# RDG0818/MAZero

Hardware: NVIDIA B200
Metric: mcts_sims_per_sec (higher is better)
Workload: dtype bf16

## Files before the change

### mazero_b200/csrc/infer_hmma.cuh

```cuda
#pragma once
#include <cuda_bf16.h>

#include "../../include/maz_infer.h"
#include "umma.cuh"

namespace maz {
namespace hmma {

using namespace umma;

constexpr int H = 128, NHEAD = 8, HD = 16, GH = 64, PH = 32, SUP = 11, NLAYER = 3;
constexpr int NCHUNK = MAZ_INFER_NCHUNK, NSLOT = 3;
constexpr int TM = 32;
#ifndef MAZ_HMMA_NQ
#define MAZ_HMMA_NQ 4
#endif
constexpr int NQ = MAZ_HMMA_NQ;
constexpr int NT = H / NQ / 8;
constexpr int GT = GH / NQ / 8;
constexpr int CW = H / NQ, FW = GH / NQ;
static_assert(NQ == 4 || NQ == 8, "NQ");
constexpr int NCONS = 64 * NQ, NTHREADS = NCONS + 32;
constexpr int PAD = 8;
constexpr int LDA = (H + PAD) * 2;
constexpr int LDQ = (3 * H + PAD) * 2;
constexpr int LDP = (PH + PAD) * 2;
constexpr int LDO = (48 + PAD) * 2;
constexpr int LDG = GH + 4;
constexpr int LDV = GH + 4;
constexpr uint32_t SLOT_BYTES = 128 * (H + PAD) * 2;
#ifndef MAZ_HMMA_PIECE
#define MAZ_HMMA_PIECE 4352
#endif
constexpr uint32_t PIECE = MAZ_HMMA_PIECE;
#ifndef MAZ_GEMM_UNROLL
#define MAZ_GEMM_UNROLL 2
#endif
constexpr int GEMM_UNROLL = MAZ_GEMM_UNROLL;

constexpr uint32_t OFF_X = 0;
constexpr uint32_t OFF_T = OFF_X + TM * LDA;
constexpr uint32_t OFF_HH = OFF_T + TM * LDA;
constexpr uint32_t OFF_ONE = OFF_HH + TM * LDA;
constexpr uint32_t OFF_PH = OFF_ONE + TM * LDO;
constexpr uint32_t OFF_Q = OFF_PH + TM * LDP;
constexpr uint32_t OFF_STAT = OFF_Q + TM * LDQ;
constexpr uint32_t STAT_SET = TM * NQ * 8;
constexpr uint32_t OFF_VP = OFF_STAT + 3 * TM * NQ * 8;
constexpr uint32_t OFF_ROW = OFF_VP + 2 * SUP * LDV * 4;
constexpr uint32_t OFF_W = ((OFF_ROW + TM * 16 + 127) / 128) * 128;
constexpr uint32_t OFF_P = OFF_W + NSLOT * SLOT_BYTES;
constexpr int G_R = 0, G_V = TM * LDG;
constexpr int Y_R = 0, Y_V = TM * GH;
constexpr int PL0 = 2 * TM * LDG;
static_assert((PL0 + TM * 48) * 4 <= TM * LDQ, "heads scratch must fit in the q|k|v region");
static_assert(2 * TM * GH * 4 <= 2 * TM * LDA, "layer-2 features must fit in the X + T tiles");

using Desc = ::maz_infer_desc;

struct RowInfo { int root, agent, valid, r0; };

__device__ __forceinline__ int tile_rpt(const Desc &d) { return d.roots_per_tile > 0 ? d.roots_per_tile : TM / d.N; }

struct SimIo {
    const int *idx_x;
    const int *actions;
    float *reward, *value, *probs, *beta;
    int root0;
    float *next_hidden;
    int *greedy;
    float *logits_out;
};
__device__ __forceinline__ SimIo io_from_desc(const Desc &d)
{
    return SimIo{d.idx_x, d.actions, d.reward, d.value, d.probs, d.beta, 0, d.next_hidden, d.greedy, d.logits_out};
}

__host__ __device__ inline size_t smem_bytes(int vec_floats) { return (size_t)OFF_P + (size_t)vec_floats * 4 + 128; }

#define HSM_DECL extern __shared__ __align__(128) uint8_t hsm[]
__device__ __forceinline__ uint32_t sbase()
{
    HSM_DECL;
    return smem_u32(hsm);
}

__device__ __forceinline__ void ldsm4(uint32_t addr, uint32_t (&r)[4])
{
    asm volatile("ldmatrix.sync.aligned.m8n8.x4.shared.b16 {%0,%1,%2,%3}, [%4];" : "=r"(r[0]), "=r"(r[1]), "=r"(r[2]), "=r"(r[3]) : "r"(addr));
}
__device__ __forceinline__ void mma16816(float (&c)[4], const uint32_t (&a)[4], uint32_t b0, uint32_t b1)
{
    asm volatile("mma.sync.aligned.m16n8k16.row.col.f32.bf16.bf16.f32 {%0,%1,%2,%3}, {%4,%5,%6,%7}, {%8,%9}, {%0,%1,%2,%3};"
                 : "+f"(c[0]), "+f"(c[1]), "+f"(c[2]), "+f"(c[3])
                 : "r"(a[0]), "r"(a[1]), "r"(a[2]), "r"(a[3]), "r"(b0), "r"(b1));
}
__device__ __forceinline__ uint32_t pack2(float a, float b)
{
    __nv_bfloat162 p = __floats2bfloat162_rn(a, b);
    return *reinterpret_cast<uint32_t *>(&p);
}
__device__ __forceinline__ void sts32(uint32_t saddr, uint32_t v) { asm volatile("st.shared.b32 [%0], %1;" ::"r"(saddr), "r"(v) : "memory"); }
__device__ __forceinline__ float2 ldp2(uint32_t saddr)
{
    float2 v;
    asm("ld.shared.v2.f32 {%0,%1}, [%2];" : "=f"(v.x), "=f"(v.y) : "r"(saddr));
    return v;
}
__device__ __forceinline__ float4 lds4v(uint32_t saddr)
{
    float4 v;
    asm volatile("ld.shared.v4.f32 {%0,%1,%2,%3}, [%4];" : "=f"(v.x), "=f"(v.y), "=f"(v.z), "=f"(v.w) : "r"(saddr) : "memory");
    return v;
}

struct Thr {
    int lane, warp, g, t, mt, nq, rA, rB;
    uint32_t a_off, w_off;
    __device__ __forceinline__ Thr()
    {
        const int tid = threadIdx.x;
        lane = tid & 31; warp = tid >> 5; g = lane >> 2; t = lane & 3; mt = warp & 1; nq = warp >> 1;
        rA = 16 * mt + g; rB = rA + 8;
        a_off = (uint32_t)(16 * mt + (lane & 7) + ((lane >> 3) & 1) * 8);
        w_off = (uint32_t)((lane & 7) + (lane >> 4) * 8);
    }
    __device__ __forceinline__ uint32_t a_addr(uint32_t tile, int lda) const { return tile + a_off * lda + (uint32_t)(lane >> 4) * 16u; }
    __device__ __forceinline__ uint32_t w_addr(uint32_t slot, int ldw, int n0) const
    {
        return slot + (uint32_t)(n0 + w_off) * ldw + (uint32_t)((lane >> 3) & 1) * 16u;
    }
};

template <int NT, int KS>
__device__ __forceinline__ void gemm_fixed(float (&acc)[NT][4], const Thr &th, uint32_t a_tile, int lda, uint32_t w_slot, int ldw, int n0)
{
    const uint32_t aa = th.a_addr(a_tile, lda), wa = th.w_addr(w_slot, ldw, n0);
    uint32_t a[2][4], b[2][NT / 2][4];
    ldsm4(aa, a[0]);
#pragma unroll
    for (int p = 0; p < NT / 2; ++p) ldsm4(wa + (uint32_t)(16 * p) * ldw, b[0][p]);
#pragma unroll GEMM_UNROLL
    for (int ks = 0; ks < KS; ++ks) {
        const int cur = ks & 1, nxt = cur ^ 1;
        if (ks + 1 < KS) {
            ldsm4(aa + 32u * (ks + 1), a[nxt]);
#pragma unroll
            for (int p = 0; p < NT / 2; ++p) ldsm4(wa + (uint32_t)(16 * p) * ldw + 32u * (ks + 1), b[nxt][p]);
        }
#pragma unroll
        for (int p = 0; p < NT / 2; ++p) {
            mma16816(acc[2 * p], a[cur], b[cur][p][0], b[cur][p][1]);
            mma16816(acc[2 * p + 1], a[cur], b[cur][p][2], b[cur][p][3]);
        }
    }
}
template <int NT>
__device__ __forceinline__ void gemm_rt(float (&acc)[NT][4], const Thr &th, uint32_t a_tile, int lda, uint32_t w_slot, int ldw, int n0, int K)
{
    const uint32_t aa = th.a_addr(a_tile, lda), wa = th.w_addr(w_slot, ldw, n0);
#pragma unroll 1
    for (int k0 = 0; k0 < K; k0 += 16) {
        uint32_t a[4], b[NT / 2][4];
        ldsm4(aa + 2u * k0, a);
#pragma unroll
        for (int p = 0; p < NT / 2; ++p) ldsm4(wa + (uint32_t)(16 * p) * ldw + 2u * k0, b[p]);
#pragma unroll
        for (int p = 0; p < NT / 2; ++p) {
            mma16816(acc[2 * p], a, b[p][0], b[p][1]);
            mma16816(acc[2 * p + 1], a, b[p][2], b[p][3]);
        }
    }
}

__device__ __forceinline__ void issue_chunk(const Desc &d, int k, int slot, uint64_t *bar_full)
{
    HSM_DECL;
    const uint32_t nbytes = (d.dbg_flags & 4) ? 16u : d.chunk_bytes[k];
    const uint8_t *src = reinterpret_cast<const uint8_t *>(d.wpk) + d.chunk_off[k];
    uint8_t *dst = hsm + OFF_W + (size_t)slot * SLOT_BYTES;
    mbar_expect_tx(&bar_full[slot], nbytes);
    for (uint32_t o = 0; o < nbytes; o += PIECE) {
        const uint32_t n = (nbytes - o < PIECE) ? (nbytes - o) : PIECE;
        bulk_g2s(dst + o, src + o, n, &bar_full[slot]);
    }
}

struct Ring {
    uint64_t *full, *empty;
    int c;
    __device__ __forceinline__ uint32_t acquire(int ahead = 0)
    {
        const int cc = c + ahead, s = cc % NSLOT;
        mbar_wait(&full[s], (cc / NSLOT) & 1);
        return sbase() + OFF_W + (uint32_t)s * SLOT_BYTES;
    }
    __device__ __forceinline__ void release(int lane, int n = 1)
    {
        __syncwarp();
        if (lane == 0)
            for (int i = 0; i < n; ++i) mbar_arrive(&empty[(c + i) % NSLOT]);
        c += n;
    }
};

__device__ __forceinline__ void cta_sync() { named_bar_sync(1, NCONS); }

template <int NT>
__device__ __forceinline__ void zero(float (&acc)[NT][4])
{
#pragma unroll
    for (int i = 0; i < NT; ++i) acc[i][0] = acc[i][1] = acc[i][2] = acc[i][3] = 0.f;
}
template <int NT>
__device__ __forceinline__ void copy(float (&dst)[NT][4], const float (&src)[NT][4])
{
#pragma unroll
    for (int i = 0; i < NT; ++i) { dst[i][0] = src[i][0]; dst[i][1] = src[i][1]; dst[i][2] = src[i][2]; dst[i][3] = src[i][3]; }
}

template <int NT>
__device__ __forceinline__ void add_bias(float (&acc)[NT][4], const Thr &th, uint32_t b, int n0)
{
#pragma unroll
    for (int nt = 0; nt < NT; ++nt) {
        const float2 v = ldp2(b + 4u * (n0 + 8 * nt + 2 * th.t));
        acc[nt][0] += v.x; acc[nt][1] += v.y; acc[nt][2] += v.x; acc[nt][3] += v.y;
    }
}
template <int NT>
__device__ __forceinline__ void store_tile(uint32_t tile, int ld, const Thr &th, int n0, const float (&acc)[NT][4])
{
#pragma unroll
    for (int nt = 0; nt < NT; ++nt) {
        const int c = n0 + 8 * nt + 2 * th.t;
        sts32(tile + (uint32_t)th.rA * ld + 2u * c, pack2(acc[nt][0], acc[nt][1]));
        sts32(tile + (uint32_t)th.rB * ld + 2u * c, pack2(acc[nt][2], acc[nt][3]));
    }
}
template <int NT>
__device__ __forceinline__ void relu(float (&acc)[NT][4])
{
#pragma unroll
    for (int nt = 0; nt < NT; ++nt) {
        acc[nt][0] = fmaxf(acc[nt][0], 0.f); acc[nt][1] = fmaxf(acc[nt][1], 0.f);
        acc[nt][2] = fmaxf(acc[nt][2], 0.f); acc[nt][3] = fmaxf(acc[nt][3], 0.f);
    }
}

template <int NT>
__device__ __forceinline__ void stats_write(const float (&v)[NT][4], const Thr &th, uint32_t stat)
{
    float s0 = 0.f, q0 = 0.f, s1 = 0.f, q1 = 0.f;
#pragma unroll
    for (int nt = 0; nt < NT; ++nt) {
        s0 += v[nt][0] + v[nt][1]; q0 += v[nt][0] * v[nt][0] + v[nt][1] * v[nt][1];
        s1 += v[nt][2] + v[nt][3]; q1 += v[nt][2] * v[nt][2] + v[nt][3] * v[nt][3];
    }
#pragma unroll
    for (int o = 1; o <= 2; o <<= 1) {
        s0 += __shfl_xor_sync(0xffffffffu, s0, o); q0 += __shfl_xor_sync(0xffffffffu, q0, o);
        s1 += __shfl_xor_sync(0xffffffffu, s1, o); q1 += __shfl_xor_sync(0xffffffffu, q1, o);
    }
    if (th.t == 0) {
        sts2f(stat + (uint32_t)(th.rA * NQ + th.nq) * 8u, s0, q0);
        sts2f(stat + (uint32_t)(th.rB * NQ + th.nq) * 8u, s1, q1);
    }
}
__device__ __forceinline__ void stats_read(uint32_t stat, int row, float inv_width, float &mean, float &rstd)
{
    float4 v[NQ / 2];
#pragma unroll
    for (int i = 0; i < NQ / 2; ++i) v[i] = lds4v(stat + (uint32_t)row * (NQ * 8u) + 16u * i);
    float s = 0.f, q = 0.f;
#pragma unroll
    for (int i = 0; i < NQ / 2; ++i) { s += v[i].x + v[i].z; q += v[i].y + v[i].w; }
    mean = s * inv_width;
    rstd = rsqrtf(fmaxf(q * inv_width - mean * mean, 0.f) + 1e-5f);
}

__device__ __forceinline__ void layer_norm128(float (&x)[NT][4], const Thr &th, uint32_t gam, uint32_t bet, int n0, bool relu_after)
{
    const uint32_t stat = sbase() + OFF_STAT;
    stats_write<NT>(x, th, stat);
    cta_sync();
    float mA, sA, mB, sB;
    stats_read(stat, th.rA, 1.f / H, mA, sA);
    stats_read(stat, th.rB, 1.f / H, mB, sB);
#pragma unroll
    for (int nt = 0; nt < NT; ++nt) {
        const int c = n0 + 8 * nt + 2 * th.t;
        const float2 gg = ldp2(gam + 4u * c), bb = ldp2(bet + 4u * c);
        x[nt][0] = (x[nt][0] - mA) * sA * gg.x + bb.x; x[nt][1] = (x[nt][1] - mA) * sA * gg.y + bb.y;
        x[nt][2] = (x[nt][2] - mB) * sB * gg.x + bb.x; x[nt][3] = (x[nt][3] - mB) * sB * gg.y + bb.y;
    }
    if (relu_after) relu<NT>(x);
}

__device__ __forceinline__ RowInfo row_info(int r)
{
    uint32_t a, b, c, e;
    lds4u(sbase() + OFF_ROW + 16u * r, a, b, c, e);
    RowInfo ri;
    ri.root = (int)a; ri.agent = (int)b; ri.valid = (int)c; ri.r0 = (int)e;
    return ri;
}

static __device__ __noinline__ void stage_gather(const Desc &d, const SimIo io)
{
    HSM_DECL;
    const int tid = threadIdx.x, r = tid >> 3, part = tid & 7;
    if (tid >= TM * 8) return;
    const RowInfo ri = row_info(r);
    uint32_t w[8] = {0, 0, 0, 0, 0, 0, 0, 0};
    int action = -1;
    if (ri.valid) {
        const int ix = io.idx_x ? __ldcg(io.idx_x + ri.root) : 0;
        if (d.greedy_pool == nullptr || d.cur < 0)
            action = __ldcg(io.actions + (size_t)ri.root * d.N + ri.agent);
        else if (ri.agent == d.cur)
            action = __ldcg(io.actions + ri.root);
        else if (ri.agent < d.cur)
            action = d.factor ? __ldcg(d.factor + (size_t)ri.root * d.N + ri.agent) : 0;
        else
            action = __ldcg(d.greedy_pool + ((size_t)ix * d.B + ri.root) * d.N + ri.agent);
        const float *h = d.pool + ((size_t)ix * d.B + ri.root) * (size_t)(d.N * H) + (size_t)ri.agent * H + part * 16;
#pragma unroll
        for (int i = 0; i < 4; ++i) {
            const float4 v = __ldcg(reinterpret_cast<const float4 *>(h) + i);
            w[2 * i] = pack2(v.x, v.y);
            w[2 * i + 1] = pack2(v.z, v.w);
        }
    }
    uint4 *dst = reinterpret_cast<uint4 *>(hsm + OFF_HH + (size_t)r * LDA + part * 32);
    dst[0] = make_uint4(w[0], w[1], w[2], w[3]);
    dst[1] = make_uint4(w[4], w[5], w[6], w[7]);
    if (part * 8 < d.KA) {
        const int c0 = part * 8;
        uint32_t o[4];
#pragma unroll
        for (int i = 0; i < 4; ++i) o[i] = pack2((c0 + 2 * i == action) ? 1.f : 0.f, (c0 + 2 * i + 1 == action) ? 1.f : 0.f);
        *reinterpret_cast<uint4 *>(hsm + OFF_ONE + (size_t)r * LDO + c0 * 2) = make_uint4(o[0], o[1], o[2], o[3]);
    }
}

static __device__ __noinline__ void stage_inproj(const Desc &d, Ring &ring, float (&xio)[NT][4])
{
    const Thr th;
    const uint32_t sb = sbase();
    const int n0 = CW * th.nq, ldo = (d.KA + PAD) * 2;
    float x[NT][4];
    zero<NT>(x);
    uint32_t w = ring.acquire();
    gemm_fixed<NT, 8>(x, th, sb + OFF_HH, LDA, w, LDA, n0);
    ring.release(th.lane);
    w = ring.acquire();
    gemm_rt<NT>(x, th, sb + OFF_ONE, LDO, w, ldo, n0, d.KA);
    ring.release(th.lane);
    add_bias<NT>(x, th, sb + OFF_P + 4u * d.o_bin, n0);
    const uint32_t pA = sb + OFF_P + 4u * (d.o_pos + row_info(th.rA).agent * H), pB = sb + OFF_P + 4u * (d.o_pos + row_info(th.rB).agent * H);
#pragma unroll
    for (int nt = 0; nt < NT; ++nt) {
        const int c = n0 + 8 * nt + 2 * th.t;
        const float2 a = ldp2(pA + 4u * c), b = ldp2(pB + 4u * c);
        x[nt][0] = fmaxf(x[nt][0], 0.f) + a.x; x[nt][1] = fmaxf(x[nt][1], 0.f) + a.y;
        x[nt][2] = fmaxf(x[nt][2], 0.f) + b.x; x[nt][3] = fmaxf(x[nt][3], 0.f) + b.y;
    }
    store_tile<NT>(sb + OFF_X, LDA, th, n0, x);
    copy<NT>(xio, x);
    cta_sync();
}

static __device__ __noinline__ void stage_qkv(Ring &ring, uint32_t lv)
{
    const Thr th;
    const uint32_t sb = sbase();
    const int n0 = CW * th.nq;
    float acc[3 * NT][4];
    zero<3 * NT>(acc);
    uint32_t wa[3];
#pragma unroll
    for (int i = 0; i < 3; ++i) wa[i] = th.w_addr(ring.acquire(i), LDA, n0);
    const uint32_t aa = th.a_addr(sb + OFF_X, LDA);
    constexpr int PW = NT / 2, NP = 3 * PW;
    uint32_t a[2][4], b[2][NP][4];
    ldsm4(aa, a[0]);
#pragma unroll
    for (int p = 0; p < NP; ++p) ldsm4(wa[p / PW] + (uint32_t)(16 * (p % PW)) * LDA, b[0][p]);
#pragma unroll GEMM_UNROLL
    for (int ks = 0; ks < 8; ++ks) {
        const int cur = ks & 1, nxt = cur ^ 1;
        if (ks + 1 < 8) {
            ldsm4(aa + 32u * (ks + 1), a[nxt]);
#pragma unroll
            for (int p = 0; p < NP; ++p) ldsm4(wa[p / PW] + (uint32_t)(16 * (p % PW)) * LDA + 32u * (ks + 1), b[nxt][p]);
        }
#pragma unroll
        for (int p = 0; p < NP; ++p) {
            mma16816(acc[2 * p], a[cur], b[cur][p][0], b[cur][p][1]);
            mma16816(acc[2 * p + 1], a[cur], b[cur][p][2], b[cur][p][3]);
        }
    }
    ring.release(th.lane, 3);
#pragma unroll
    for (int which = 0; which < 3; ++which) {
#pragma unroll
        for (int nt = 0; nt < NT; ++nt) {
            const int c = n0 + 8 * nt + 2 * th.t;
            const float2 bv = ldp2(lv + 4u * (which * H + c));
            const float *v = acc[which * NT + nt];
            sts32(sb + OFF_Q + (uint32_t)th.rA * LDQ + 2u * (which * H + c), pack2(v[0] + bv.x, v[1] + bv.y));
            sts32(sb + OFF_Q + (uint32_t)th.rB * LDQ + 2u * (which * H + c), pack2(v[2] + bv.x, v[3] + bv.y));
        }
    }
    cta_sync();
}

__device__ __forceinline__ void unpack16(const uint32_t (&w)[8], float (&f)[16])
{
#pragma unroll
    for (int i = 0; i < 8; ++i) {
        f[2 * i] = __uint_as_float(w[i] << 16);
        f[2 * i + 1] = __uint_as_float(w[i] & 0xffff0000u);
    }
}
__device__ __forceinline__ void lds32B(uint32_t saddr, uint32_t (&w)[8])
{
    lds4u(saddr, w[0], w[1], w[2], w[3]);
    lds4u(saddr + 16u, w[4], w[5], w[6], w[7]);
}

template <int NN>
__device__ __forceinline__ void attention_small(uint32_t qbase, int r0, int hh, const float (&q)[16], float (&o)[16])
{
    float s[NN];
    uint32_t kw[NN][8], vw[NN][8];
#pragma unroll
    for (int j = 0; j < NN; ++j) {
        const uint32_t kr = qbase + (uint32_t)(r0 + j) * LDQ + H * 2 + hh * 32;
        lds32B(kr, kw[j]);
        lds32B(kr + H * 2, vw[j]);
    }
#pragma unroll
    for (int j = 0; j < NN; ++j) {
        float k[16];
        unpack16(kw[j], k);
        float a = 0.f, b = 0.f;
#pragma unroll
        for (int i = 0; i < 16; i += 2) { a += q[i] * k[i]; b += q[i + 1] * k[i + 1]; }
        s[j] = a + b;
    }
    float m = s[0];
#pragma unroll
    for (int j = 1; j < NN; ++j) m = fmaxf(m, s[j]);
    float l = 0.f;
#pragma unroll
    for (int j = 0; j < NN; ++j) { s[j] = __expf(s[j] - m); l += s[j]; }
    const float inv = 1.f / l;
#pragma unroll
    for (int i = 0; i < 16; ++i) o[i] = 0.f;
#pragma unroll
    for (int j = 0; j < NN; ++j) {
        float v[16];
        unpack16(vw[j], v);
        const float p = s[j] * inv;
#pragma unroll
        for (int i = 0; i < 16; ++i) o[i] += p * v[i];
    }
}

static __device__ __noinline__ void stage_attention(const Desc &d)
{
    const uint32_t sb = sbase(), qbase = sb + OFF_Q;
    const int tid = threadIdx.x, r = tid >> 3, hh = tid & 7;
    if (tid >= TM * NHEAD) {
        cta_sync();
        return;
    }
    const RowInfo ri = row_info(r);
    const int N = d.N;
    float q[16], o[16];
    {
        uint32_t w[8];
        lds32B(qbase + (uint32_t)r * LDQ + hh * 32, w);
        unpack16(w, q);
#pragma unroll
        for (int i = 0; i < 16; ++i) q[i] *= 0.25f;
    }
    if (N <= 4) {
        switch (N) {
            case 1: attention_small<1>(qbase, ri.r0, hh, q, o); break;
            case 2: attention_small<2>(qbase, ri.r0, hh, q, o); break;
            case 3: attention_small<3>(qbase, ri.r0, hh, q, o); break;
            default: attention_small<4>(qbase, ri.r0, hh, q, o); break;
        }
    } else {
#pragma unroll
        for (int i = 0; i < 16; ++i) o[i] = 0.f;
        float m = -INFINITY, lsum = 0.f;
#pragma unroll 1
        for (int j = 0; j < N; ++j) {
            const uint32_t kr = qbase + (uint32_t)(ri.r0 + j) * LDQ + H * 2 + hh * 32;
            uint32_t kw[8], vw[8];
            lds32B(kr, kw);
            lds32B(kr + H * 2, vw);
            float k[16], v[16];
            unpack16(kw, k);
            unpack16(vw, v);
            float s = 0.f;
#pragma unroll
            for (int i = 0; i < 16; ++i) s += q[i] * k[i];
            const float mn = fmaxf(m, s);
            const float corr = __expf(m - mn), p = __expf(s - mn);
            lsum = lsum * corr + p;
#pragma unroll
            for (int i = 0; i < 16; ++i) o[i] = o[i] * corr + p * v[i];
            m = mn;
        }
        const float inv = 1.f / lsum;
#pragma unroll
        for (int i = 0; i < 16; ++i) o[i] *= inv;
    }
    uint4 a, b;
    a.x = pack2(o[0], o[1]); a.y = pack2(o[2], o[3]); a.z = pack2(o[4], o[5]); a.w = pack2(o[6], o[7]);
    b.x = pack2(o[8], o[9]); b.y = pack2(o[10], o[11]); b.z = pack2(o[12], o[13]); b.w = pack2(o[14], o[15]);
    sts4(sb + OFF_T + (uint32_t)r * LDA + hh * 32, a);
    sts4(sb + OFF_T + (uint32_t)r * LDA + hh * 32 + 16, b);
    cta_sync();
}

static __device__ __noinline__ void stage_residual_ln(Ring &ring, float (&xio)[NT][4], uint32_t bias, uint32_t gam, uint32_t bet)
{
    const Thr th;
    const uint32_t sb = sbase();
    const int n0 = CW * th.nq;
    float x[NT][4];
    copy<NT>(x, xio);
    const uint32_t w = ring.acquire();
    gemm_fixed<NT, 8>(x, th, sb + OFF_T, LDA, w, LDA, n0);
    ring.release(th.lane);
    add_bias<NT>(x, th, bias, n0);
    layer_norm128(x, th, gam, bet, n0, false);
    store_tile<NT>(sb + OFF_X, LDA, th, n0, x);
    copy<NT>(xio, x);
    cta_sync();
}

static __device__ __noinline__ void stage_linear_relu(Ring &ring, uint32_t bias)
{
    const Thr th;
    const uint32_t sb = sbase();
    const int n0 = CW * th.nq;
    float acc[NT][4];
    zero<NT>(acc);
    const uint32_t w = ring.acquire();
    gemm_fixed<NT, 8>(acc, th, sb + OFF_X, LDA, w, LDA, n0);
    ring.release(th.lane);
    add_bias<NT>(acc, th, bias, n0);
    relu<NT>(acc);
    store_tile<NT>(sb + OFF_T, LDA, th, n0, acc);
    cta_sync();
}

static __device__ __noinline__ void stage_dynamics(const Desc &d, Ring &ring, const SimIo io)
{
    const Thr th;
    const uint32_t sb = sbase();
    const int n0 = CW * th.nq, ldo = (d.KA + PAD) * 2;
    const uint32_t dv = sb + OFF_P + 4u * d.o_dyn;
    float acc[NT][4];
    zero<NT>(acc);
    uint32_t w = ring.acquire();
    gemm_fixed<NT, 8>(acc, th, sb + OFF_HH, LDA, w, LDA, n0);
    ring.release(th.lane);
    w = ring.acquire();
    gemm_rt<NT>(acc, th, sb + OFF_ONE, LDO, w, ldo, n0, d.KA);
    ring.release(th.lane);
    w = ring.acquire();
    gemm_fixed<NT, 8>(acc, th, sb + OFF_X, LDA, w, LDA, n0);
    ring.release(th.lane);
    add_bias<NT>(acc, th, dv, n0);
    layer_norm128(acc, th, dv + 4u * 128, dv + 4u * 256, n0, true);
    store_tile<NT>(sb + OFF_T, LDA, th, n0, acc);
    cta_sync();
    zero<NT>(acc);
    w = ring.acquire();
    gemm_fixed<NT, 8>(acc, th, sb + OFF_T, LDA, w, LDA, n0);
    ring.release(th.lane);
    add_bias<NT>(acc, th, dv + 4u * 384, n0);
    layer_norm128(acc, th, dv + 4u * 512, dv + 4u * 640, n0, true);
    store_tile<NT>(sb + OFF_X, LDA, th, n0, acc);
    cta_sync();
    const RowInfo ra = row_info(th.rA), rb = row_info(th.rB);
    float2 hv[2][NT];
#pragma unroll
    for (int hf = 0; hf < 2; ++hf) {
        const RowInfo &ri = hf ? rb : ra;
        const int ix = (ri.valid && io.idx_x) ? io.idx_x[ri.root - io.root0] : 0;
        const float *hp = d.pool + ((size_t)ix * d.B + (ri.valid ? ri.root : 0)) * (size_t)(d.N * H) + (size_t)ri.agent * H;
#pragma unroll
        for (int nt = 0; nt < NT; ++nt)
            hv[hf][nt] = ri.valid ? __ldcg(reinterpret_cast<const float2 *>(hp + n0 + 8 * nt + 2 * th.t)) : make_float2(0.f, 0.f);
    }
    zero<NT>(acc);
    w = ring.acquire();
    gemm_fixed<NT, 8>(acc, th, sb + OFF_X, LDA, w, LDA, n0);
    ring.release(th.lane);
    add_bias<NT>(acc, th, dv + 4u * 768, n0);
#pragma unroll
    for (int hf = 0; hf < 2; ++hf) {
        const RowInfo &ri = hf ? rb : ra;
        float *nh = io.next_hidden + (size_t)(ri.valid ? ri.root : 0) * (d.N * H) + (size_t)ri.agent * H;
#pragma unroll
        for (int nt = 0; nt < NT; ++nt) {
            acc[nt][2 * hf] += hv[hf][nt].x;
            acc[nt][2 * hf + 1] += hv[hf][nt].y;
            if (ri.valid) *reinterpret_cast<float2 *>(nh + n0 + 8 * nt + 2 * th.t) = make_float2(acc[nt][2 * hf], acc[nt][2 * hf + 1]);
        }
    }
    store_tile<NT>(sb + OFF_T, LDA, th, n0, acc);
    cta_sync();
}

__device__ __forceinline__ void gnn_phase_a(const float (&acc)[NT][4], const Thr &th, uint32_t G, uint32_t b)
{
    const int f0 = FW * th.nq + 2 * th.t;
#pragma unroll
    for (int tl = 0; tl < GT; ++tl) {
        const float2 bg = ldp2(b + 4u * (f0 + 8 * tl));
        sts2f(G + 4u * (th.rA * LDG + f0 + 8 * tl), acc[tl][0] + bg.x, acc[tl][1] + bg.y);
        sts2f(G + 4u * (th.rB * LDG + f0 + 8 * tl), acc[tl][2] + bg.x, acc[tl][3] + bg.y);
    }
}
template <int NN>
__device__ __forceinline__ void agent_sums(uint32_t G, int f0, int r0A, int r0B, float2 (&sa)[GT], float2 (&sc)[GT])
{
    float2 a[NN][GT], c[NN][GT];
#pragma unroll
    for (int j = 0; j < NN; ++j)
#pragma unroll
        for (int tl = 0; tl < GT; ++tl) {
            a[j][tl] = lds2f(G + 4u * ((r0A + j) * LDG + f0 + 8 * tl));
            c[j][tl] = lds2f(G + 4u * ((r0B + j) * LDG + f0 + 8 * tl));
        }
#pragma unroll
    for (int j = 0; j < NN; ++j)
#pragma unroll
        for (int tl = 0; tl < GT; ++tl) {
            sa[tl].x += a[j][tl].x; sa[tl].y += a[j][tl].y; sc[tl].x += c[j][tl].x; sc[tl].y += c[j][tl].y;
        }
}
__device__ __forceinline__ void gnn_phase_b(const float (&acc)[NT][4], const Thr &th, uint32_t G, uint32_t b, uint32_t stat, int N, int r0A,
                                            int r0B, float (&y)[GT][4])
{
    const int f0 = FW * th.nq + 2 * th.t;
    float2 sa[GT], sc[GT];
#pragma unroll
    for (int tl = 0; tl < GT; ++tl) sa[tl] = sc[tl] = make_float2(0.f, 0.f);
    {
        int j = 0;
#pragma unroll 1
        for (; j + 3 <= N; j += 3) agent_sums<3>(G, f0, r0A + j, r0B + j, sa, sc);
#pragma unroll 1
        for (; j < N; ++j) agent_sums<1>(G, f0, r0A + j, r0B + j, sa, sc);
    }
#pragma unroll
    for (int tl = 0; tl < GT; ++tl) {
        const float2 bn = ldp2(b + 4u * (GH + f0 + 8 * tl));
        y[tl][0] = fmaxf(sa[tl].x + acc[GT + tl][0] + bn.x, 0.f); y[tl][1] = fmaxf(sa[tl].y + acc[GT + tl][1] + bn.y, 0.f);
        y[tl][2] = fmaxf(sc[tl].x + acc[GT + tl][2] + bn.x, 0.f); y[tl][3] = fmaxf(sc[tl].y + acc[GT + tl][3] + bn.y, 0.f);
    }
    stats_write<GT>(y, th, stat);
}
__device__ __forceinline__ void gnn_phase_c(const Thr &th, uint32_t stat, float (&y)[GT][4])
{
    float mA, sA, mB, sB;
    stats_read(stat, th.rA, 1.f / GH, mA, sA);
    stats_read(stat, th.rB, 1.f / GH, mB, sB);
#pragma unroll
    for (int tl = 0; tl < GT; ++tl) {
        y[tl][0] = (y[tl][0] - mA) * sA; y[tl][1] = (y[tl][1] - mA) * sA;
        y[tl][2] = (y[tl][2] - mB) * sB; y[tl][3] = (y[tl][3] - mB) * sB;
    }
}

static __device__ __noinline__ void stage_heads1(const Desc &d, Ring &ring)
{
    const Thr th;
    const uint32_t sb = sbase();
    const int n0 = CW * th.nq, ldo = (d.KA + PAD) * 2;
    float aR[NT][4], aV[NT][4], aP[2][4];
    zero<NT>(aR); zero<NT>(aV); zero<2>(aP);
    uint32_t w = ring.acquire();
    gemm_fixed<NT, 8>(aR, th, sb + OFF_T, LDA, w, LDA, n0);
    ring.release(th.lane);
    w = ring.acquire();
    gemm_rt<NT>(aR, th, sb + OFF_ONE, LDO, w, ldo, n0, d.KA);
    ring.release(th.lane);
    w = ring.acquire();
    gemm_fixed<NT, 8>(aV, th, sb + OFF_T, LDA, w, LDA, n0);
    ring.release(th.lane);
    w = ring.acquire();
    if (th.nq < 2) gemm_fixed<2, 8>(aP, th, sb + OFF_T, LDA, w, LDA, 16 * th.nq);
    ring.release(th.lane);
    const uint32_t G = sb + OFF_Q, stat = sb + OFF_STAT, pr = sb + OFF_P + 4u * d.o_rg, pvv = sb + OFF_P + 4u * d.o_vg;
    const uint32_t pp = sb + OFF_P + 4u * d.o_pol;
    gnn_phase_a(aR, th, G + 4u * G_R, pr);
    gnn_phase_a(aV, th, G + 4u * G_V, pvv);
    if (th.nq < 2) add_bias<2>(aP, th, pp, 16 * th.nq);
    stats_write<2>(aP, th, stat + 2 * STAT_SET);
    cta_sync();
    const int r0A = row_info(th.rA).r0, r0B = row_info(th.rB).r0;
    float yR[GT][4], yV[GT][4];
    gnn_phase_b(aR, th, G + 4u * G_R, pr, stat, d.N, r0A, r0B, yR);
    gnn_phase_b(aV, th, G + 4u * G_V, pvv, stat + STAT_SET, d.N, r0A, r0B, yV);
    if (th.nq < 2) {
        float mA, sA, mB, sB;
        stats_read(stat + 2 * STAT_SET, th.rA, 1.f / PH, mA, sA);
        stats_read(stat + 2 * STAT_SET, th.rB, 1.f / PH, mB, sB);
#pragma unroll
        for (int tl = 0; tl < 2; ++tl) {
            const int c = 16 * th.nq + 8 * tl + 2 * th.t;
            const float2 gg = ldp2(pp + 4u * (PH + c)), bb = ldp2(pp + 4u * (2 * PH + c));
            const float v0 = fmaxf((aP[tl][0] - mA) * sA * gg.x + bb.x, 0.f), v1 = fmaxf((aP[tl][1] - mA) * sA * gg.y + bb.y, 0.f);
            const float v2 = fmaxf((aP[tl][2] - mB) * sB * gg.x + bb.x, 0.f), v3 = fmaxf((aP[tl][3] - mB) * sB * gg.y + bb.y, 0.f);
            sts32(sb + OFF_PH + (uint32_t)th.rA * LDP + 2u * c, pack2(v0, v1));
            sts32(sb + OFF_PH + (uint32_t)th.rB * LDP + 2u * c, pack2(v2, v3));
        }
    }
    cta_sync();
    gnn_phase_c(th, stat, yR);
    gnn_phase_c(th, stat + STAT_SET, yV);
    store_tile<GT>(sb + OFF_X, LDA, th, FW * th.nq, yR);
    store_tile<GT>(sb + OFF_X, LDA, th, GH + FW * th.nq, yV);
    cta_sync();
}

__device__ __forceinline__ float support_to_scalar(const float (&v)[SUP])
{
    float m = v[0];
#pragma unroll
    for (int k = 1; k < SUP; ++k) m = fmaxf(m, v[k]);
    float s = 0.f, x = 0.f;
#pragma unroll
    for (int k = 0; k < SUP; ++k) {
        const float e = __expf(v[k] - m);
        s += e;
        x += e * (float)(k - 5);
    }
    x /= s;
    const float eps = 0.001f;
    const float r = (sqrtf(1.f + 4.f * eps * (fabsf(x) + 1.f + eps)) - 1.f) / (2.f * eps);
    float out = r * r - 1.f;
    out = (x < 0.f) ? -out : out;
    if (!(out == out)) out = 0.f;
    if (fabsf(out) < eps) out = 0.f;
    return out;
}

static __device__ __noinline__ void stage_heads2(const Desc &d, Ring &ring, const SimIo io, long long *hs_clk)
{
    const Thr th;
    const uint32_t sb = sbase();
    const int n0 = CW * th.nq, ldg = (GH + PAD) * 2;
    const int N = d.N, A = d.A, tid = threadIdx.x;
    int hs_n = 40;
#define HS() \
    if (hs_clk && hs_n < 64) hs_clk[hs_n++] = clock64();
    HS();
    float aR[NT][4], aV[NT][4], aP[2][4];
    zero<NT>(aR); zero<NT>(aV); zero<2>(aP);
    uint32_t w = ring.acquire();
    gemm_fixed<NT, 4>(aR, th, sb + OFF_X, LDA, w, ldg, n0);
    ring.release(th.lane);
    w = ring.acquire();
    gemm_fixed<NT, 4>(aV, th, sb + OFF_X + GH * 2, LDA, w, ldg, n0);
    ring.release(th.lane);
    w = ring.acquire();
    const int pc0 = 16 * th.nq;
    if (pc0 < d.NAP) gemm_fixed<2, 2>(aP, th, sb + OFF_PH, LDP, w, LDP, pc0);
    ring.release(th.lane);
    const uint32_t G = sb + OFF_Q, stat = sb + OFF_STAT, pr = sb + OFF_P + 4u * (d.o_rg + 128), pvv = sb + OFF_P + 4u * (d.o_vg + 128);
    const uint32_t PL = G + 4u * PL0;
    HS();
    gnn_phase_a(aR, th, G + 4u * G_R, pr);
    gnn_phase_a(aV, th, G + 4u * G_V, pvv);
    if (pc0 < d.NAP) {
        const uint32_t b2 = sb + OFF_P + 4u * (d.o_pol + 96);
#pragma unroll
        for (int tl = 0; tl < 2; ++tl) {
            const int c = pc0 + 8 * tl + 2 * th.t;
            const float2 bb = ldp2(b2 + 4u * c);
            sts2f(PL + 4u * (th.rA * 48 + c), aP[tl][0] + bb.x, aP[tl][1] + bb.y);
            sts2f(PL + 4u * (th.rB * 48 + c), aP[tl][2] + bb.x, aP[tl][3] + bb.y);
        }
    }
    cta_sync();
    HS();
    const int r0A = row_info(th.rA).r0, r0B = row_info(th.rB).r0;
    float yR[GT][4], yV[GT][4];
    gnn_phase_b(aR, th, G + 4u * G_R, pr, stat, N, r0A, r0B, yR);
    gnn_phase_b(aV, th, G + 4u * G_V, pvv, stat + STAT_SET, N, r0A, r0B, yV);
    const uint32_t YB = sb + OFF_X;
#pragma unroll
    for (int tl = 0; tl < GT; ++tl) {
        const int f = FW * th.nq + 8 * tl + 2 * th.t;
        sts2f(YB + 4u * (Y_R + th.rA * GH + f), yR[tl][0], yR[tl][1]);
        sts2f(YB + 4u * (Y_R + th.rB * GH + f), yR[tl][2], yR[tl][3]);
        sts2f(YB + 4u * (Y_V + th.rA * GH + f), yV[tl][0], yV[tl][1]);
        sts2f(YB + 4u * (Y_V + th.rB * GH + f), yV[tl][2], yV[tl][3]);
    }
    HS();
    if (tid < TM * 8) {
        constexpr int PA = 6;
        const int r = tid >> 3, sub = tid & 7;
        const RowInfo ri = row_info(r);
        const uint32_t lg = PL + 4u * (r * 48);
        float v[PA];
#pragma unroll
        for (int i = 0; i < PA; ++i) v[i] = (sub + 8 * i < A) ? lds1v(lg + 4u * (sub + 8 * i)) : -INFINITY;
        float m = -INFINITY;
        int am = 0x7fffffff;
#pragma unroll
        for (int i = 0; i < PA; ++i)
            if (v[i] > m) { m = v[i]; am = sub + 8 * i; }
#pragma unroll
        for (int o = 1; o <= 4; o <<= 1) {
            const float om = __shfl_xor_sync(0xffffffffu, m, o);
            const int oa = __shfl_xor_sync(0xffffffffu, am, o);
            if (om > m || (om == m && oa < am)) { m = om; am = oa; }
        }
        HS();
        const bool unit_tau = (d.inv_tau == 1.0f);
        float e[PA], eb[PA], s = 0.f, sbeta = 0.f;
#pragma unroll
        for (int i = 0; i < PA; ++i) {
            e[i] = (sub + 8 * i < A) ? __expf(v[i] - m) : 0.f;
            eb[i] = unit_tau ? e[i] : ((sub + 8 * i < A) ? __powf(e[i], d.inv_tau) : 0.f);
            s += e[i];
            sbeta += eb[i];
        }
#pragma unroll
        for (int o = 1; o <= 4; o <<= 1) {
            s += __shfl_xor_sync(0xffffffffu, s, o);
            sbeta += __shfl_xor_sync(0xffffffffu, sbeta, o);
        }
        HS();
        if (ri.valid) {
            if (io.greedy && sub == 0) io.greedy[(size_t)ri.root * N + ri.agent] = am;
            const int ta = (d.cur < 0) ? ri.agent : (ri.agent == d.cur ? 0 : -1);
            const float invs = 1.f / s, invb = 1.f / sbeta;
#pragma unroll
            for (int i = 0; i < PA; ++i) {
                const int a = sub + 8 * i;
                if (a < A) {
                    if (io.logits_out) io.logits_out[((size_t)ri.root * N + ri.agent) * A + a] = v[i];
                    if (ta >= 0) {
                        const size_t o = ((size_t)(ri.root - io.root0) * d.Nt + ta) * A + a;
                        io.probs[o] = e[i] * invs;
                        io.beta[o] = eb[i] * invb;
                    }
                }
            }
        }
    }
    HS();
    cta_sync();
    HS();
    const int rpt = tile_rpt(d);
    const uint32_t POOL = G;
    const float invn = 1.f / (float)N;
    for (int i = tid; i < 2 * rpt * (GH / 2); i += NCONS) {
        const int f2 = i & (GH / 2 - 1), rest = i >> 5, kind = rest >= rpt ? 1 : 0, rl = rest - kind * rpt;
        const uint32_t src = YB + 4u * ((kind ? Y_V : Y_R) + (rl * N) * GH + 2 * f2), st = stat + (kind ? STAT_SET : 0u);
        float2 s = make_float2(0.f, 0.f);
        int j = 0;
#pragma unroll 1
        for (; j + 3 <= N; j += 3) {
            float m0, r0, m1, r1, m2, r2;
            stats_read(st, rl * N + j, 1.f / GH, m0, r0);
            stats_read(st, rl * N + j + 1, 1.f / GH, m1, r1);
            stats_read(st, rl * N + j + 2, 1.f / GH, m2, r2);
            const float2 v0 = lds2f(src + 4u * (j * GH)), v1 = lds2f(src + 4u * ((j + 1) * GH)), v2 = lds2f(src + 4u * ((j + 2) * GH));
            s.x += (v0.x - m0) * r0 + (v1.x - m1) * r1 + (v2.x - m2) * r2;
            s.y += (v0.y - m0) * r0 + (v1.y - m1) * r1 + (v2.y - m2) * r2;
        }
#pragma unroll 1
        for (; j < N; ++j) {
            float m0, r0;
            stats_read(st, rl * N + j, 1.f / GH, m0, r0);
            const float2 v = lds2f(src + 4u * (j * GH));
            s.x += (v.x - m0) * r0; s.y += (v.y - m0) * r0;
        }
        sts2f(POOL + 4u * ((kind * rpt + rl) * GH + 2 * f2), s.x * invn, s.y * invn);
    }
    cta_sync();
    HS();
    {
        const int hw = tid >> 4, l16 = tid & 15, lane = tid & 31;
        for (int pair = hw; pair < rpt * 2; pair += NCONS / 16) {
            const int rl = pair >> 1, kind = pair & 1;
            float logit = 0.f;
            if (l16 < SUP) {
                const uint32_t pv = POOL + 4u * ((kind * rpt + rl) * GH), vw = sb + OFF_VP + 4u * ((kind * SUP + l16) * LDV);
                float s0 = 0.f, s1 = 0.f;
#pragma unroll
                for (int f = 0; f < GH; f += 32) {
                    float4 a[8], wv[8];
#pragma unroll
                    for (int q = 0; q < 8; ++q) a[q] = lds4v(pv + 4u * (f + 4 * q));
#pragma unroll
                    for (int q = 0; q < 8; ++q) wv[q] = lds4(vw + 4u * (f + 4 * q));
#pragma unroll
                    for (int q = 0; q < 8; q += 2) {
                        s0 += a[q].x * wv[q].x + a[q].y * wv[q].y + a[q].z * wv[q].z + a[q].w * wv[q].w;
                        s1 += a[q + 1].x * wv[q + 1].x + a[q + 1].y * wv[q + 1].y + a[q + 1].z * wv[q + 1].z + a[q + 1].w * wv[q + 1].w;
                    }
                }
                logit = s0 + s1 + lds1(sb + OFF_P + 4u * ((kind ? d.o_vg : d.o_rg) + 256 + SUP * GH + l16));
            }
            float v[SUP];
#pragma unroll
            for (int k = 0; k < SUP; ++k) v[k] = __shfl_sync(0xffffffffu, logit, (lane & 16) + k);
            const int root = blockIdx.x * rpt + rl;
            if (l16 == 0 && root < d.B) (kind ? io.value : io.reward)[root - io.root0] = support_to_scalar(v);
        }
    }
    HS();
#undef HS
}

__device__ __forceinline__ void setup_rows(const Desc &d)
{
    HSM_DECL;
    const int tid = threadIdx.x, N = d.N;
    if (tid < TM) {
        const int rpt = tile_rpt(d), rl = tid / N, agent = tid - rl * N;
        const int root = blockIdx.x * rpt + rl;
        RowInfo ri;
        ri.valid = (rl < rpt) && (root < d.B);
        ri.root = root; ri.agent = (rl < rpt) ? agent : 0;
        ri.r0 = (rl < rpt) ? rl * N : 0;
        reinterpret_cast<RowInfo *>(hsm + OFF_ROW)[tid] = ri;
    }
}

__device__ __forceinline__ void produce_weights(const Desc &d, uint64_t *bar_full, uint64_t *bar_empty, uint64_t *bar_vec, int rounds)
{
    HSM_DECL;
    mbar_expect_tx(bar_vec, (uint32_t)d.vec_floats * 4u);
    bulk_g2s(hsm + OFF_P, d.vec, (uint32_t)d.vec_floats * 4u, bar_vec);
    const int total = rounds * NCHUNK;
#pragma unroll 1
    for (int c = 0, k = 0; c < total; ++c, k = (k + 1 == NCHUNK) ? 0 : k + 1) {
        const int s = c % NSLOT;
        if (c >= NSLOT) mbar_wait_backoff(&bar_empty[s], ((c / NSLOT) - 1) & 1);
        issue_chunk(d, k, s, bar_full);
    }
}

__device__ __forceinline__ void setup_head_copies(const Desc &d)
{
    const uint32_t sb = sbase();
    for (int i = threadIdx.x; i < 2 * SUP * GH; i += NCONS) {
        const int f = i % GH, rest = i / GH, k = rest % SUP, kind = rest / SUP;
        sts1f(sb + OFF_VP + 4u * ((kind * SUP + k) * LDV + f), lds1v(sb + OFF_P + 4u * ((kind ? d.o_vg : d.o_rg) + 256 + k * GH + f)));
    }
}

__device__ __forceinline__ void infer_stages(const Desc &d, const SimIo io, Ring &ring, long long *clk)
{
    int ts_n = 2;
#define TS() \
    if (clk && ts_n < 64) clk[ts_n++] = clock64();
    TS();
    float x[NT][4];
    stage_inproj(d, ring, x);
    TS();
    const uint32_t pbase = sbase() + OFF_P;
#pragma unroll 1
    for (int l = 0; l < NLAYER; ++l) {
        const uint32_t lv = pbase + 4u * (d.o_layer + l * 1280);
        stage_qkv(ring, lv);
        TS();
        stage_attention(d);
        TS();
        stage_residual_ln(ring, x, lv + 4u * 384, lv + 4u * 512, lv + 4u * 640);
        TS();
        stage_linear_relu(ring, lv + 4u * 768);
        TS();
        stage_residual_ln(ring, x, lv + 4u * 896, lv + 4u * 1024, lv + 4u * 1152);
        TS();
    }
    TS();
    stage_dynamics(d, ring, io);
    TS();
    stage_heads1(d, ring);
    TS();
    stage_heads2(d, ring, io, clk);
    TS();
#undef TS
}

#ifndef MAZ_HMMA_NO_KERNEL
__global__ void __launch_bounds__(NTHREADS, 1) k_recurrent_inference_small(const __grid_constant__ Desc d)
{
    HSM_DECL;
    __shared__ __align__(8) uint64_t bar_full[NSLOT], bar_empty[NSLOT], bar_vec;
    const int tid = threadIdx.x, warp = tid >> 5;

    if (tid == 0) {
        for (int i = 0; i < NSLOT; ++i) { mbar_init(&bar_full[i], 1); mbar_init(&bar_empty[i], NCONS / 32); }
        mbar_init(&bar_vec, 1);
        mbar_fence_init();
    }
    setup_rows(d);
    __syncthreads();

    if (warp == NCONS / 32) {
        if ((tid & 31) == 0) produce_weights(d, bar_full, bar_empty, &bar_vec, 1);
        return;
    }
    Ring ring{bar_full, bar_empty, 0};
    long long *clk = (d.dbg_clock != nullptr && blockIdx.x == 0 && tid == 0) ? d.dbg_clock : nullptr;
    if (clk) clk[0] = clock64();
    asm volatile("griddepcontrol.wait;" ::: "memory");
    asm volatile("griddepcontrol.launch_dependents;" ::: "memory");
    const SimIo io = io_from_desc(d);
    stage_gather(d, io);
    if (clk) clk[1] = clock64();
    mbar_wait(&bar_vec, 0);
    setup_head_copies(d);
    cta_sync();
    infer_stages(d, io, ring, clk);
}
#endif

}
}
```

### mazero_b200/csrc/maz_infer.cu

```cuda
#include <cuda_bf16.h>
#include <cuda_runtime.h>

#include <string>

#include "../../include/maz_infer.h"
#include "umma.cuh"
#include "infer_fused.cuh"
#include "infer_hmma.cuh"
#include "infer_twin.cuh"

using namespace maz;
using namespace maz::umma;

extern "C" const char *maz_last_error(void);
namespace maz { int set_last_error(int code, const std::string &msg); bool pdl_enabled(); int pdl_mask(); }

__global__ void __launch_bounds__(128, 1) k_dbg_umma_gemm(const float *__restrict__ a, const __nv_bfloat16 *__restrict__ wp,
                                                          float *__restrict__ out, int N, int K)
{
    extern __shared__ __align__(1024) uint8_t smem[];
    __shared__ __align__(8) uint64_t bar_w, bar_mma;
    __shared__ uint32_t tmem_base_s;
    uint8_t *sA = smem + ((1024u - (smem_u32(smem) & 1023u)) & 1023u);
    uint8_t *sW = smem + operand_bytes(128, K);
    const int tid = threadIdx.x, warp = tid >> 5;

    if (tid == 0) {
        mbar_init(&bar_w, 1);
        mbar_init(&bar_mma, 1);
        mbar_fence_init();
    }
    if (warp == 0) tmem_alloc(&tmem_base_s, 256);
    tc_fence_before();
    __syncthreads();
    tc_fence_after();
    const uint32_t tmem_base = tmem_base_s;

    if (tid == 0) {
        mbar_expect_tx(&bar_w, operand_bytes(N, K));
        bulk_g2s(sW, wp, operand_bytes(N, K), &bar_w);
    }
    for (int k8 = 0; k8 < K / 8; ++k8) {
        const float4 lo = *reinterpret_cast<const float4 *>(a + (size_t)tid * K + k8 * 8);
        const float4 hi = *reinterpret_cast<const float4 *>(a + (size_t)tid * K + k8 * 8 + 4);
        __nv_bfloat162 p0 = __floats2bfloat162_rn(lo.x, lo.y), p1 = __floats2bfloat162_rn(lo.z, lo.w);
        __nv_bfloat162 p2 = __floats2bfloat162_rn(hi.x, hi.y), p3 = __floats2bfloat162_rn(hi.z, hi.w);
        uint4 v;
        v.x = *reinterpret_cast<uint32_t *>(&p0);
        v.y = *reinterpret_cast<uint32_t *>(&p1);
        v.z = *reinterpret_cast<uint32_t *>(&p2);
        v.w = *reinterpret_cast<uint32_t *>(&p3);
        *reinterpret_cast<uint4 *>(sA + operand_chunk_off(tid, k8, K, 128)) = v;
    }
    fence_proxy_async();
    __syncthreads();
    if (tid == 0) {
        mbar_wait(&bar_w, 0);
        tc_fence_after();
        issue_gemm(tmem_base, smem_u32(sA), K, 0, smem_u32(sW), K, 0, K, N, false);
        mma_commit(&bar_mma);
    }
    mbar_wait(&bar_mma, 0);
    tc_fence_after();
    const uint32_t lane_base = tmem_base + ((uint32_t)(warp * 32) << 16);
    for (int c = 0; c < N; c += 16) {
        float v[16];
        tmem_ld16(lane_base + c, v);
#pragma unroll
        for (int i = 0; i < 16; ++i) out[(size_t)tid * N + c + i] = v[i];
    }
    tc_fence_before();
    __syncthreads();
    if (warp == 0) tmem_dealloc(tmem_base, 256);
}

extern "C" int maz_dbg_umma_gemm(const float *a, const void *w_packed, float *out, int n, int k, void *stream)
{
    if (!a || !w_packed || !out || n % 16 || k % 16 || n < 16 || n > 256 || k < 16 || k > 512)
        return set_last_error(1, "maz_dbg_umma_gemm: bad arguments");
    const size_t dyn = operand_bytes(128, k) + operand_bytes(n, k) + 2048;
    cudaError_t e = cudaFuncSetAttribute(k_dbg_umma_gemm, cudaFuncAttributeMaxDynamicSharedMemorySize, (int)dyn);
    if (e != cudaSuccess) return set_last_error(2, std::string("cudaFuncSetAttribute: ") + cudaGetErrorString(e));
    k_dbg_umma_gemm<<<1, 128, dyn, static_cast<cudaStream_t>(stream)>>>(a, static_cast<const __nv_bfloat16 *>(w_packed), out, n, k);
    e = cudaGetLastError();
    if (e != cudaSuccess) return set_last_error(2, std::string("k_dbg_umma_gemm: ") + cudaGetErrorString(e));
    return 0;
}

extern "C" int maz_infer_configure(int vec_floats, int ka);

extern "C" int maz_infer_recurrent(const maz_infer_desc *d, void *stream)
{
    if (!d) return set_last_error(1, "maz_infer_recurrent: NULL descriptor");
    if (d->B <= 0 || d->N <= 0 || d->N > 32 || d->A <= 0 || d->A > 48 || d->KA % 16 || d->KA < d->A || d->NAP != d->KA)
        return set_last_error(3, "maz_infer_recurrent: unsupported shape (agents <= 32, actions <= 48)");
    if (!d->pool || !d->actions || !d->next_hidden || !d->reward || !d->value || !d->probs || !d->beta || !d->wpk || !d->vec)
        return set_last_error(1, "maz_infer_recurrent: NULL tensor");
    if (d->vec_floats <= 0 || d->vec_floats % 4) return set_last_error(1, "maz_infer_recurrent: vec_floats must be a positive multiple of 4");
    const bool tw = d->tc_layout == 1;
    if (d->tc_layout != 0 && !tw) return set_last_error(1, "maz_infer_recurrent: unknown tc_layout");
    if (tw && (d->o_oh_in <= 0 || d->o_oh_dyn <= 0 || d->o_oh_rg <= 0 || d->o_oh_rg + d->A * 64 > d->vec_floats))
        return set_last_error(1, "maz_infer_recurrent: tc_layout 1 needs the one-hot weight tables behind vec");
    const size_t dyn = tw ? twin::smem_bytes() : fused::smem_bytes(d->KA, d->vec_floats);
    if (dyn > 227 * 1024) return set_last_error(3, "maz_infer_recurrent: parameters do not fit in shared memory");
    if (int rc = maz_infer_configure(d->vec_floats, d->KA)) return rc;
    const int roots_per_tile = 4 * (32 / d->N);
    int tiles = (d->B + roots_per_tile - 1) / roots_per_tile;
    if (tw) tiles = (tiles + 1) / 2;
    cudaLaunchConfig_t cfg = {};
    cfg.gridDim = dim3((unsigned)tiles);
    cfg.blockDim = dim3(fused::NTHREADS);
    cfg.dynamicSmemBytes = dyn;
    cfg.stream = static_cast<cudaStream_t>(stream);
    cudaLaunchAttribute attr[1];
    attr[0].id = cudaLaunchAttributeProgrammaticStreamSerialization;
    attr[0].val.programmaticStreamSerializationAllowed = 1;
    cfg.attrs = attr;
    cfg.numAttrs = (maz::pdl_mask() & 1) ? 1 : 0;
    cudaError_t e = tw ? cudaLaunchKernelEx(&cfg, twin::k_recurrent_inference_twin, *d) : cudaLaunchKernelEx(&cfg, fused::k_recurrent_inference, *d);
    if (e != cudaSuccess) return set_last_error(2, std::string("k_recurrent_inference: ") + cudaGetErrorString(e));
    return 0;
}

extern "C" int maz_infer_small_nq(void) { return hmma::NQ; }

extern "C" int maz_infer_configure(int vec_floats, int ka)
{
    (void)vec_floats; (void)ka;
    static bool done[64] = {};
    int dev = 0;
    if (cudaGetDevice(&dev) != cudaSuccess) return set_last_error(2, "no CUDA device available (libmaz_b200 has no CPU fallback)");
    if (dev < 0 || dev >= 64 || done[dev]) return 0;
    int optin = 227 * 1024;
    cudaDeviceGetAttribute(&optin, cudaDevAttrMaxSharedMemoryPerBlockOptin, dev);
    cudaFuncAttributes fa;
    cudaError_t e = cudaFuncGetAttributes(&fa, hmma::k_recurrent_inference_small);
    if (e == cudaSuccess)
        e = cudaFuncSetAttribute(hmma::k_recurrent_inference_small, cudaFuncAttributeMaxDynamicSharedMemorySize, optin - (int)fa.sharedSizeBytes);
    if (e == cudaSuccess) e = cudaFuncGetAttributes(&fa, fused::k_recurrent_inference);
    if (e == cudaSuccess)
        e = cudaFuncSetAttribute(fused::k_recurrent_inference, cudaFuncAttributeMaxDynamicSharedMemorySize, optin - (int)fa.sharedSizeBytes);
    if (e == cudaSuccess) e = cudaFuncGetAttributes(&fa, twin::k_recurrent_inference_twin);
    if (e == cudaSuccess)
        e = cudaFuncSetAttribute(twin::k_recurrent_inference_twin, cudaFuncAttributeMaxDynamicSharedMemorySize, optin - (int)fa.sharedSizeBytes);
    if (e != cudaSuccess) return set_last_error(2, std::string("cudaFuncSetAttribute: ") + cudaGetErrorString(e));
    done[dev] = true;
    return 0;
}

extern "C" int maz_infer_recurrent_small(const maz_infer_desc *d, void *stream)
{
    if (!d) return set_last_error(1, "maz_infer_recurrent_small: NULL descriptor");
    if (d->B <= 0 || d->N <= 0 || d->N > 32 || d->A <= 0 || d->A > 48 || d->KA % 16 || d->KA < d->A || d->NAP != d->KA)
        return set_last_error(3, "maz_infer_recurrent_small: unsupported shape (agents <= 32, actions <= 48)");
    if (!d->pool || !d->actions || !d->next_hidden || !d->reward || !d->value || !d->probs || !d->beta || !d->wpk || !d->vec)
        return set_last_error(1, "maz_infer_recurrent_small: NULL tensor");
    if (d->vec_floats <= 0 || d->vec_floats % 4) return set_last_error(1, "maz_infer_recurrent_small: vec_floats must be a positive multiple of 4");
    for (int c = 0; c < MAZ_INFER_NCHUNK; ++c)
        if (d->chunk_bytes[c] == 0 || d->chunk_bytes[c] > hmma::SLOT_BYTES || d->chunk_bytes[c] % 16 || d->chunk_off[c] % 16)
            return set_last_error(1, "maz_infer_recurrent_small: bad weight chunk table");
    const size_t dyn = hmma::smem_bytes(d->vec_floats);
    if (dyn > 227 * 1024) return set_last_error(3, "maz_infer_recurrent_small: parameters do not fit in shared memory");
    if (int rc = maz_infer_configure(d->vec_floats, d->KA)) return rc;
    const int rpt = hmma::TM / d->N;
    const int tiles = (d->B + rpt - 1) / rpt;
    cudaLaunchConfig_t cfg = {};
    cfg.gridDim = dim3((unsigned)tiles);
    cfg.blockDim = dim3(hmma::NTHREADS);
    cfg.dynamicSmemBytes = dyn;
    cfg.stream = static_cast<cudaStream_t>(stream);
    cudaLaunchAttribute attr[1];
    attr[0].id = cudaLaunchAttributeProgrammaticStreamSerialization;
    attr[0].val.programmaticStreamSerializationAllowed = 1;
    cfg.attrs = attr;
    cfg.numAttrs = (maz::pdl_mask() & 1) ? 1 : 0;
    cudaError_t e = cudaLaunchKernelEx(&cfg, hmma::k_recurrent_inference_small, *d);
    if (e != cudaSuccess) return set_last_error(2, std::string("k_recurrent_inference_small: ") + cudaGetErrorString(e));
    return 0;
}
```

### mazero_b200/csrc/maz_search.cu

```cuda
#include <cuda_runtime.h>

#include <cstdlib>
#include <cstring>
#include <string>
#include <vector>

#include "../../include/maz_search.h"
#include "../../include/maz_turn.h"
#define MAZ_HMMA_NO_KERNEL
#include "search_persist.cuh"
#include "tree_host.h"

using namespace maz;

#define CU_TRY(expr)                                                                                          \
    do {                                                                                                      \
        cudaError_t e__ = (expr);                                                                             \
        if (e__ != cudaSuccess)                                                                               \
            return set_last_error(MAZ_ERR_CUDA, std::string(#expr) + ": " + cudaGetErrorString(e__));         \
    } while (0)
#define MAZ_TRY(expr)          \
    do {                       \
        int rc__ = (expr);     \
        if (rc__) return rc__; \
    } while (0)

namespace {

struct DevGuard {
    int prev = -1;
    explicit DevGuard(int dev)
    {
        if (cudaGetDevice(&prev) != cudaSuccess) prev = -1;
        if (prev != dev) cudaSetDevice(dev);
    }
    ~DevGuard()
    {
        if (prev >= 0) cudaSetDevice(prev);
    }
};

struct GraphKey {
    int cur;
    float inv_tau, c_base, c_init, discount, delta_lb, rho, lam;
    bool operator==(const GraphKey &o) const { return std::memcmp(this, &o, sizeof(GraphKey)) == 0; }
};
struct GraphEntry {
    GraphKey key;
    cudaGraphExec_t exec;
    unsigned long long used;
};
constexpr size_t kMaxGraphs = 40;

}

struct maz_search {
    maz_search_config cfg{};
    maz_infer_desc tc{}, sm{};
    maz_mlp_desc mlp{};
    int Nt = 1, D = 0, rpt = 1, strategy = MAZ_SEARCH_GRAPH;
    bool use_small = false;
    cudaStream_t stream = nullptr, cap_stream = nullptr;
    maz_tree *tree = nullptr;
    bool own_pool = false;
    float *pool = nullptr;
    int *greedy = nullptr;
    int *idx_x = nullptr, *idx_y = nullptr, *act = nullptr, *factor = nullptr;
    float *sim_r = nullptr, *sim_v = nullptr, *sim_p = nullptr, *sim_b = nullptr;
    float *root_p = nullptr, *root_b = nullptr, *root_n = nullptr;
    size_t bytes = 0;
    float *rec_r = nullptr, *rec_v = nullptr, *rec_p = nullptr, *rec_b = nullptr;
    int *rec_ix = nullptr, *rec_act = nullptr;
    long long *dbg_clock = nullptr;
    cudaEvent_t ev0 = nullptr, ev1 = nullptr;
    bool timing = false, timed = false;
    std::vector<GraphEntry> graphs;
    unsigned long long tick = 0;
    char *h_in = nullptr, *d_in = nullptr, *h_out = nullptr, *d_out = nullptr;
    size_t in_bytes = 0, out_bytes = 0;
};

static int dmalloc(maz_search *s, void **p, size_t bytes)
{
    CU_TRY(cudaMalloc(p, bytes));
    s->bytes += bytes;
    return MAZ_OK;
}

static int env_strategy()
{
    const char *e = getenv("MAZ_SEARCH_STRATEGY");
    if (!e) return MAZ_SEARCH_AUTO;
    if (!strcmp(e, "persistent")) return MAZ_SEARCH_PERSISTENT;
    if (!strcmp(e, "graph")) return MAZ_SEARCH_GRAPH;
    return MAZ_SEARCH_AUTO;
}
static int env_int(const char *name, int dflt)
{
    const char *e = getenv(name);
    return e ? atoi(e) : dflt;
}

extern "C" {

int maz_search_create(maz_search **out, const maz_search_config *cfg)
{
    if (!out || !cfg) return set_last_error(MAZ_ERR_INVALID, "maz_search_create: NULL argument");
    *out = nullptr;
    if (cfg->B <= 0 || cfg->N <= 0 || cfg->A <= 0 || cfg->K <= 0 || cfg->S <= 0 || cfg->hidden <= 0)
        return set_last_error(MAZ_ERR_INVALID, "maz_search_create: dimensions must be positive");
    if (cfg->net_kind == MAZ_NET_SMAC && (!cfg->smac_tc || !cfg->smac_small || cfg->hidden != hmma::H))
        return set_last_error(MAZ_ERR_INVALID, "maz_search_create: MAZ_NET_SMAC needs both weight packings and hidden 128");
    if (cfg->net_kind == MAZ_NET_MLP && !cfg->mlp) return set_last_error(MAZ_ERR_INVALID, "maz_search_create: MAZ_NET_MLP needs the MLP descriptor");
    if (cfg->net_kind != MAZ_NET_SMAC && cfg->net_kind != MAZ_NET_MLP) return set_last_error(MAZ_ERR_INVALID, "maz_search_create: bad net_kind");
    int ndev = 0;
    if (cudaGetDeviceCount(&ndev) != cudaSuccess || ndev == 0)
        return set_last_error(MAZ_ERR_CUDA, "no CUDA device available (libmaz_b200 has no CPU fallback)");
    if (cfg->device < 0 || cfg->device >= ndev) return set_last_error(MAZ_ERR_INVALID, "maz_search_create: bad device index");
    DevGuard g(cfg->device);

    maz_search *s = new maz_search();
    s->cfg = *cfg;
    if (cfg->net_kind == MAZ_NET_SMAC) { s->tc = *cfg->smac_tc; s->sm = *cfg->smac_small; }
    else s->mlp = *cfg->mlp;
    s->cfg.smac_tc = s->cfg.smac_small = nullptr;
    s->cfg.mlp = nullptr;
    const int B = cfg->B, N = cfg->N, A = cfg->A, K = cfg->K, S = cfg->S;
    s->Nt = cfg->joint ? N : 1;
    s->D = N * cfg->hidden;
    auto fail = [&](int rc) { std::string m = maz_last_error(); maz_search_destroy(s); set_last_error(rc, m); return rc; };

    int rc = maz_tree_create_ex(&s->tree, B, s->Nt, A, K, S, 0.01f, 0u, 0.75f, 0.8f, cfg->device, 0u);
    if (rc) return fail(rc);
    s->bytes += maz_tree_arena_bytes(s->tree);

    int sms = 148;
    cudaDeviceGetAttribute(&sms, cudaDevAttrMultiProcessorCount, cfg->device);
    int strat = cfg->strategy != MAZ_SEARCH_AUTO ? cfg->strategy : env_strategy();
    const int rpt_fit = hmma::TM / N;
    int rpt = rpt_fit < 8 ? rpt_fit : 8;
    const int rpt_env = env_int("MAZ_SEARCH_RPT", 0);
    if (rpt_env > 0 && rpt_env < rpt) rpt = rpt_env;
    int optin = 227 * 1024;
    cudaDeviceGetAttribute(&optin, cudaDevAttrMaxSharedMemoryPerBlockOptin, cfg->device);
    bool persist_ok = cfg->net_kind == MAZ_NET_SMAC && N <= hmma::TM && rpt >= 1 &&
                      (size_t)rpt * tree_scratch_bytes(s->Nt, A, K, S) <= persist::TREE_SCRATCH_BYTES &&
                      persist::persist_smem_bytes(s->sm.vec_floats, rpt, s->Nt, A, S) + 256 <= (size_t)optin;
    if (strat == MAZ_SEARCH_PERSISTENT && !persist_ok) {
        set_last_error(MAZ_ERR_UNSUPPORTED, "maz_search_create: the persistent kernel does not support this network / shape");
        return fail(MAZ_ERR_UNSUPPORTED);
    }
    {
        const char *k = getenv("MAZ_INFER_KERNEL");
        if (strat == MAZ_SEARCH_AUTO && k && !strcmp(k, "tcgen05")) strat = MAZ_SEARCH_GRAPH;
    }
    if (strat == MAZ_SEARCH_AUTO) {
        const int waves_max = env_int("MAZ_SEARCH_PERSIST_MAX_CTAS", sms);
        strat = (persist_ok && (B + rpt - 1) / rpt <= waves_max) ? MAZ_SEARCH_PERSISTENT : MAZ_SEARCH_GRAPH;
    }
    s->strategy = strat;
    s->rpt = rpt;
    if (cfg->net_kind == MAZ_NET_SMAC) {
        const char *k = getenv("MAZ_INFER_KERNEL");
        const int small_max = env_int("MAZ_INFER_SMALL_MAX_TILES", 222);
        s->use_small = k && !strcmp(k, "small") ? true : k && !strcmp(k, "tcgen05") ? false : (B + rpt_fit - 1) / rpt_fit <= small_max;
    }

    const size_t NA = (size_t)s->Nt * A;
    if (cfg->pool) s->pool = cfg->pool;
    else {
        if ((rc = dmalloc(s, (void **)&s->pool, sizeof(float) * (size_t)(S + 1) * B * s->D))) return fail(rc);
        s->own_pool = true;
    }
    if ((rc = dmalloc(s, (void **)&s->greedy, sizeof(int) * (size_t)(S + 1) * B * N)) ||
        (rc = dmalloc(s, (void **)&s->idx_x, sizeof(int) * B)) || (rc = dmalloc(s, (void **)&s->idx_y, sizeof(int) * B)) ||
        (rc = dmalloc(s, (void **)&s->act, sizeof(int) * B * s->Nt)) || (rc = dmalloc(s, (void **)&s->factor, sizeof(int) * B * N)) ||
        (rc = dmalloc(s, (void **)&s->sim_r, sizeof(float) * B)) || (rc = dmalloc(s, (void **)&s->sim_v, sizeof(float) * B)) ||
        (rc = dmalloc(s, (void **)&s->sim_p, sizeof(float) * B * NA)) || (rc = dmalloc(s, (void **)&s->sim_b, sizeof(float) * B * NA)) ||
        (rc = dmalloc(s, (void **)&s->root_p, sizeof(float) * B * NA)) || (rc = dmalloc(s, (void **)&s->root_b, sizeof(float) * B * NA)) ||
        (rc = dmalloc(s, (void **)&s->root_n, sizeof(float) * B * NA)))
        return fail(rc);
    if (cudaMemset(s->greedy, 0, sizeof(int) * (size_t)(S + 1) * B * N) != cudaSuccess ||
        cudaMemset(s->factor, 0, sizeof(int) * B * N) != cudaSuccess) {
        set_last_error(MAZ_ERR_CUDA, "cudaMemset failed");
        return fail(MAZ_ERR_CUDA);
    }
    if (s->strategy == MAZ_SEARCH_PERSISTENT) {
        cudaFuncAttributes fa;
        cudaError_t e = cudaFuncGetAttributes(&fa, persist::k_search_persistent<false>);
        if (e == cudaSuccess)
            e = cudaFuncSetAttribute(persist::k_search_persistent<false>, cudaFuncAttributeMaxDynamicSharedMemorySize, optin - (int)fa.sharedSizeBytes);
        if (e == cudaSuccess)
            e = cudaFuncSetAttribute(persist::k_search_persistent<true>, cudaFuncAttributeMaxDynamicSharedMemorySize, optin - (int)fa.sharedSizeBytes);
        if (e != cudaSuccess) {
            set_last_error(MAZ_ERR_CUDA, std::string("cudaFuncSetAttribute(k_search_persistent): ") + cudaGetErrorString(e));
            return fail(MAZ_ERR_CUDA);
        }
        int nb = 0;
        const size_t dyn = persist::persist_smem_bytes(s->sm.vec_floats, rpt, s->Nt, A, S);
        e = cudaOccupancyMaxActiveBlocksPerMultiprocessor(&nb, persist::k_search_persistent<false>, persist::PERSIST_THREADS, dyn);
        if (e != cudaSuccess || nb < 1) {
            set_last_error(MAZ_ERR_CUDA, "k_search_persistent does not fit on an SM: " + std::to_string(fa.numRegs) + " registers x " +
                                             std::to_string(persist::PERSIST_THREADS) + " threads, " + std::to_string(dyn) + " + " +
                                             std::to_string(fa.sharedSizeBytes) + " bytes of shared memory (opt-in limit " + std::to_string(optin) + ")");
            return fail(MAZ_ERR_CUDA);
        }
    } else {
        if (cudaStreamCreateWithFlags(&s->cap_stream, cudaStreamNonBlocking) != cudaSuccess) {
            set_last_error(MAZ_ERR_CUDA, "cudaStreamCreate failed");
            return fail(MAZ_ERR_CUDA);
        }
        if (cfg->net_kind == MAZ_NET_SMAC && (rc = maz_infer_configure(s->sm.vec_floats, s->sm.KA))) return fail(rc);
    }
    *out = s;
    return MAZ_OK;
}

void maz_search_destroy(maz_search *s)
{
    if (!s) return;
    DevGuard g(s->cfg.device);
    for (auto &e : s->graphs) cudaGraphExecDestroy(e.exec);
    if (s->cap_stream) cudaStreamDestroy(s->cap_stream);
    if (s->ev0) cudaEventDestroy(s->ev0);
    if (s->ev1) cudaEventDestroy(s->ev1);
    maz_tree_destroy(s->tree);
    if (s->own_pool) cudaFree(s->pool);
    void *ptrs[] = {s->greedy, s->idx_x, s->idx_y, s->act, s->factor, s->sim_r, s->sim_v, s->sim_p, s->sim_b,
                    s->root_p, s->root_b, s->root_n, s->d_in, s->d_out};
    for (void *p : ptrs) cudaFree(p);
    if (s->h_in) cudaFreeHost(s->h_in);
    if (s->h_out) cudaFreeHost(s->h_out);
    delete s;
}

int maz_search_set_stream(maz_search *s, void *stream)
{
    if (!s) return set_last_error(MAZ_ERR_INVALID, "null handle");
    s->stream = static_cast<cudaStream_t>(stream);
    return maz_tree_set_stream(s->tree, stream);
}
int maz_search_strategy(const maz_search *s) { return s ? s->strategy : 0; }
size_t maz_search_device_bytes(const maz_search *s) { return s ? s->bytes : 0; }
float *maz_search_pool(maz_search *s) { return s ? s->pool : nullptr; }
maz_tree *maz_search_tree(maz_search *s) { return s ? s->tree : nullptr; }
int maz_search_root_arrays(maz_search *s, const float **probs, const float **beta, const float **noises)
{
    if (!s) return set_last_error(MAZ_ERR_INVALID, "null handle");
    if (probs) *probs = s->root_p;
    if (beta) *beta = s->root_b;
    if (noises) *noises = s->root_n;
    return MAZ_OK;
}
int maz_search_check(maz_search *s)
{
    if (!s) return set_last_error(MAZ_ERR_INVALID, "null handle");
    return maz_tree_check(s->tree);
}
int maz_search_set_record(maz_search *s, float *rewards, float *values, float *probs, float *beta, int *idx_x, int *actions)
{
    if (!s) return set_last_error(MAZ_ERR_INVALID, "null handle");
    if (rewards && (!values || !probs || !beta || !idx_x || !actions))
        return set_last_error(MAZ_ERR_INVALID, "maz_search_set_record: all six arrays or none");
    s->rec_r = rewards; s->rec_v = values; s->rec_p = probs; s->rec_b = beta; s->rec_ix = idx_x; s->rec_act = actions;
    return MAZ_OK;
}
int maz_search_set_debug_clock(maz_search *s, long long *p)
{
    if (!s) return set_last_error(MAZ_ERR_INVALID, "null handle");
    s->dbg_clock = p;
    return MAZ_OK;
}

int maz_search_set_timing(maz_search *s, int on)
{
    if (!s) return set_last_error(MAZ_ERR_INVALID, "null handle");
    DevGuard g(s->cfg.device);
    if (on && !s->ev0) {
        CU_TRY(cudaEventCreate(&s->ev0));
        CU_TRY(cudaEventCreate(&s->ev1));
    }
    s->timing = on != 0;
    s->timed = false;
    return MAZ_OK;
}
int maz_search_loop_ms(maz_search *s, float *ms)
{
    if (!s || !ms) return set_last_error(MAZ_ERR_INVALID, "maz_search_loop_ms: NULL argument");
    if (!s->timed) return set_last_error(MAZ_ERR_INVALID, "maz_search_loop_ms: no timed search yet (maz_search_set_timing)");
    DevGuard g(s->cfg.device);
    CU_TRY(cudaEventSynchronize(s->ev1));
    CU_TRY(cudaEventElapsedTime(ms, s->ev0, s->ev1));
    return MAZ_OK;
}
int maz_search_roots_per_cta(const maz_search *s) { return s && s->strategy == MAZ_SEARCH_PERSISTENT ? s->rpt : 0; }

}

static int launch_inference(maz_search *s, const maz_search_call *c, int sim, const int *idx_x, const int *act, float *r, float *v,
                            float *p, float *b, cudaStream_t stream)
{
    const int B = s->cfg.B, N = s->cfg.N;
    const bool seq = !s->cfg.joint;
    float *next_hidden = s->pool + (size_t)(sim + 1) * B * s->D;
    int *greedy = seq ? s->greedy + (size_t)(sim + 1) * B * N : nullptr;
    if (s->cfg.net_kind == MAZ_NET_SMAC) {
        maz_infer_desc d = s->use_small ? s->sm : s->tc;
        d.B = B; d.Nt = s->Nt; d.cur = seq ? c->cur : -1; d.inv_tau = 1.0f / c->tau;
        d.pool = s->pool; d.idx_x = idx_x; d.actions = act; d.next_hidden = next_hidden;
        d.reward = r; d.value = v; d.probs = p; d.beta = b; d.greedy = greedy; d.logits_out = nullptr;
        d.dbg_clock = nullptr; d.roots_per_tile = 0;
        d.factor = seq ? s->factor : nullptr;
        d.greedy_pool = seq ? s->greedy : nullptr;
        return s->use_small ? maz_infer_recurrent_small(&d, stream) : maz_infer_recurrent(&d, stream);
    }
    maz_mlp_desc d = s->mlp;
    d.B = B; d.Nt = s->Nt; d.cur = seq ? c->cur : -1; d.inv_tau = 1.0f / c->tau;
    d.pool = s->pool; d.idx_x = idx_x; d.actions = act; d.next_hidden = next_hidden;
    d.reward = r; d.value = v; d.probs = p; d.beta = b; d.greedy = greedy; d.logits_out = nullptr;
    d.factor = seq ? s->factor : nullptr;
    d.greedy_pool = seq ? s->greedy : nullptr;
    return maz_mlp_recurrent(&d, stream);
}

static int enqueue_loop(maz_search *s, const maz_search_call *c, cudaStream_t stream, bool record)
{
    const int B = s->cfg.B, S = s->cfg.S, K = s->cfg.K;
    const size_t NA = (size_t)s->Nt * s->cfg.A;
    maz_tree *t = s->tree;
    cudaStream_t keep = t->stream;
    t->stream = stream;
    auto slice = [&](int sim, int *&ix, int *&act, float *&r, float *&v, float *&p, float *&b) {
        const size_t o = record ? (size_t)sim : 0;
        ix = (record ? s->rec_ix : s->idx_x) + o * B;
        act = (record ? s->rec_act : s->act) + o * B * s->Nt;
        r = (record ? s->rec_r : s->sim_r) + o * B;
        v = (record ? s->rec_v : s->sim_v) + o * B;
        p = (record ? s->rec_p : s->sim_p) + o * B * NA;
        b = (record ? s->rec_b : s->sim_b) + o * B * NA;
    };
    int *ix, *act, *ixn, *actn;
    float *r, *v, *p, *b, *rn, *vn, *pn, *bn;
    slice(0, ix, act, r, v, p, b);
    int rc = maz_tree_batch_selection_dev(t, c->pb_c_base, c->pb_c_init, c->discount, ix, s->idx_y, act);
    for (int sim = 0; sim < S && !rc; ++sim) {
        rc = launch_inference(s, c, sim, ix, act, r, v, p, b, stream);
        if (rc) break;
        if (sim + 1 < S) {
            slice(sim + 1, ixn, actn, rn, vn, pn, bn);
            rc = maz_tree_expansion_backup_selection_dev(t, sim + 1, c->discount, K, r, v, p, b, c->pb_c_base, c->pb_c_init, ixn,
                                                         s->idx_y, actn);
            ix = ixn; act = actn; r = rn; v = vn; p = pn; b = bn;
        } else {
            rc = maz_tree_batch_expansion_and_backup_dev(t, sim + 1, c->discount, K, r, v, p, b);
        }
    }
    t->stream = keep;
    return rc;
}

static int graph_for(maz_search *s, const maz_search_call *c, cudaGraphExec_t *out)
{
    GraphKey key;
    std::memset(&key, 0, sizeof(key));
    key.cur = s->cfg.joint ? -1 : c->cur;
    key.inv_tau = 1.0f / c->tau; key.c_base = c->pb_c_base; key.c_init = c->pb_c_init; key.discount = c->discount;
    key.delta_lb = c->delta_lb; key.rho = c->rho; key.lam = c->lam;
    for (auto &e : s->graphs)
        if (e.key == key) {
            e.used = ++s->tick;
            *out = e.exec;
            return MAZ_OK;
        }
    cudaGraph_t graph = nullptr;
    CU_TRY(cudaStreamBeginCapture(s->cap_stream, cudaStreamCaptureModeThreadLocal));
    int rc = enqueue_loop(s, c, s->cap_stream, false);
    cudaError_t e = cudaStreamEndCapture(s->cap_stream, &graph);
    if (rc) {
        if (graph) cudaGraphDestroy(graph);
        return rc;
    }
    if (e != cudaSuccess) return set_last_error(MAZ_ERR_CUDA, std::string("cudaStreamEndCapture: ") + cudaGetErrorString(e));
    cudaGraphExec_t exec = nullptr;
    e = cudaGraphInstantiate(&exec, graph, 0);
    cudaGraphDestroy(graph);
    if (e != cudaSuccess) return set_last_error(MAZ_ERR_CUDA, std::string("cudaGraphInstantiate: ") + cudaGetErrorString(e));
    if (s->graphs.size() >= kMaxGraphs) {
        size_t lru = 0;
        for (size_t i = 1; i < s->graphs.size(); ++i)
            if (s->graphs[i].used < s->graphs[lru].used) lru = i;
        cudaGraphExecDestroy(s->graphs[lru].exec);
        s->graphs.erase(s->graphs.begin() + lru);
    }
    s->graphs.push_back(GraphEntry{key, exec, ++s->tick});
    *out = exec;
    return MAZ_OK;
}

static int launch_persistent(maz_search *s, const maz_search_call *c, bool record)
{
    const int B = s->cfg.B;
    const bool seq = !s->cfg.joint;
    maz_tree *t = s->tree;
    persist::SearchParams P;
    std::memset(&P, 0, sizeof(P));
    P.d = s->sm;
    maz_infer_desc &d = P.d;
    d.B = B; d.Nt = s->Nt; d.cur = seq ? c->cur : -1; d.inv_tau = 1.0f / c->tau;
    d.pool = s->pool; d.next_hidden = s->pool + (size_t)B * s->D;
    d.idx_x = nullptr; d.actions = nullptr;
    d.reward = d.value = d.probs = d.beta = nullptr;
    d.greedy = nullptr; d.logits_out = nullptr; d.dbg_clock = nullptr;
    d.roots_per_tile = s->rpt;
    d.factor = seq ? s->factor : nullptr;
    d.greedy_pool = seq ? s->greedy : nullptr;
    P.L = t->L;
    P.arena = t->arena;
    P.lam_pow = t->d_lam_pow; P.logterm = t->d_logterm; P.sqrtn = t->d_sqrtn; P.table_len = t->table_len;
    P.discount = c->discount; P.K = s->cfg.K; P.S = s->cfg.S;
    P.g_err = t->d_err;
    P.idx_y = s->idx_y;
    P.greedy_w = seq ? s->greedy : nullptr;
    if (record) { P.rec_r = s->rec_r; P.rec_v = s->rec_v; P.rec_p = s->rec_p; P.rec_b = s->rec_b; P.rec_ix = s->rec_ix; P.rec_act = s->rec_act; }
    P.tree_clock = s->dbg_clock;
    const unsigned grid = (unsigned)((B + s->rpt - 1) / s->rpt);
    const size_t dyn = persist::persist_smem_bytes(s->sm.vec_floats, s->rpt, s->Nt, s->cfg.A, s->cfg.S);
    if (P.tree_clock != nullptr) persist::k_search_persistent<true><<<grid, persist::PERSIST_THREADS, dyn, s->stream>>>(P);
    else persist::k_search_persistent<false><<<grid, persist::PERSIST_THREADS, dyn, s->stream>>>(P);
    CU_TRY(cudaGetLastError());
    return MAZ_OK;
}

extern "C" int maz_search_run_dev(maz_search *s, const maz_search_call *c)
{
    if (!s || !c) return set_last_error(MAZ_ERR_INVALID, "maz_search_run_dev: NULL argument");
    const int B = s->cfg.B, N = s->cfg.N, A = s->cfg.A, K = s->cfg.K;
    const bool seq = !s->cfg.joint;
    if (seq ? (c->cur < 0 || c->cur >= N) : (c->cur >= 0))
        return set_last_error(MAZ_ERR_INVALID, "maz_search_run_dev: current agent index does not match the handle's mode");
    if (!c->rewards || !c->values || !c->logits || !c->noise) return set_last_error(MAZ_ERR_INVALID, "maz_search_run_dev: NULL input");
    if (!(c->tau > 0.f)) return set_last_error(MAZ_ERR_INVALID, "maz_search_run_dev: sampled_tau must be positive");
    DevGuard g(s->cfg.device);
    cudaStream_t st = s->stream;
    if (c->root_hidden && c->root_hidden != s->pool)
        CU_TRY(cudaMemcpyAsync(s->pool, c->root_hidden, sizeof(float) * (size_t)B * s->D, cudaMemcpyDeviceToDevice, st));
    MAZ_TRY(maz_root_prepare_dev(c->logits, c->legal, c->noise, B, N, A, seq ? c->cur : -1, c->noise_eps, 1.0f / c->tau, s->root_p,
                                 s->root_b, s->root_n, s->greedy, st));
    if (seq && c->cur > 0) {
        if (c->factor) {
            if (c->factor != s->factor) CU_TRY(cudaMemcpyAsync(s->factor, c->factor, sizeof(int) * (size_t)B * N, cudaMemcpyDeviceToDevice, st));
        } else {
            CU_TRY(cudaMemsetAsync(s->factor, 0, sizeof(int) * (size_t)B * N, st));
        }
    }
    MAZ_TRY(maz_tree_set_stream(s->tree, st));
    MAZ_TRY(maz_tree_reset(s->tree, c->seed, c->delta_lb, c->rho, c->lam, c->root_index_offset));
    MAZ_TRY(maz_tree_set_puct(s->tree, c->pb_c_base, c->pb_c_init));
    MAZ_TRY(maz_tree_prepare_dev(s->tree, c->rewards, c->values, s->root_p, s->root_b, K, c->noise_eps, s->root_n));
    const bool record = s->rec_r != nullptr;
    if (s->timing) CU_TRY(cudaEventRecord(s->ev0, st));
    if (s->strategy == MAZ_SEARCH_PERSISTENT) {
        MAZ_TRY(launch_persistent(s, c, record));
    } else if (record) {
        MAZ_TRY(enqueue_loop(s, c, st, true));
    } else {
        cudaGraphExec_t exec = nullptr;
        MAZ_TRY(graph_for(s, c, &exec));
        CU_TRY(cudaGraphLaunch(exec, st));
    }
    if (s->timing) {
        CU_TRY(cudaEventRecord(s->ev1, st));
        s->timed = true;
    }
    const maz_search_readout &o = c->out;
    return maz_tree_readout_dev(s->tree, c->discount, o.values, o.marginal_visit_count, o.marginal_priors, o.num_children, o.actions,
                                o.visit_count, o.pred_probs, o.beta, o.beta_hat, o.priors, o.imp_ratio, o.pred_values, o.mcts_values,
                                o.rewards, o.qvalues);
}

extern "C" int maz_search_run(maz_search *s, const maz_search_call *c)
{
    if (!s || !c) return set_last_error(MAZ_ERR_INVALID, "maz_search_run: NULL argument");
    if (!c->root_hidden || !c->rewards || !c->values || !c->logits || !c->noise)
        return set_last_error(MAZ_ERR_INVALID, "maz_search_run: NULL input");
    DevGuard g(s->cfg.device);
    const size_t B = s->cfg.B, N = s->cfg.N, A = s->cfg.A, K = s->cfg.K, Nt = s->Nt, D = s->D;
    const size_t n_hidden = B * D, n_b = B, n_bna = B * N * A, n_noise = B * Nt * A, n_fac = B * N;
    const size_t in_words = n_hidden + 2 * n_b + 2 * n_bna + n_noise + n_fac;
    const size_t n_mv = B * Nt * A, n_act = B * K * Nt, n_k = B * K;
    const size_t out_words = n_b + 2 * n_mv + n_b + n_act + n_k + 9 * n_k;
    if (!s->h_in) {
        CU_TRY(cudaMallocHost((void **)&s->h_in, 4 * in_words));
        CU_TRY(cudaMallocHost((void **)&s->h_out, 4 * out_words));
        MAZ_TRY(dmalloc(s, (void **)&s->d_in, 4 * in_words));
        MAZ_TRY(dmalloc(s, (void **)&s->d_out, 4 * out_words));
        s->in_bytes = 4 * in_words;
        s->out_bytes = 4 * out_words;
    }
    size_t o = 0;
    auto put = [&](const void *src, size_t words) {
        const size_t at = o;
        if (src) std::memcpy(s->h_in + 4 * at, src, 4 * words);
        o += words;
        return at;
    };
    const size_t o_hid = put(c->root_hidden, n_hidden), o_r = put(c->rewards, n_b), o_v = put(c->values, n_b),
                 o_log = put(c->logits, n_bna), o_leg = put(c->legal, n_bna), o_noi = put(c->noise, n_noise), o_fac = put(c->factor, n_fac);
    CU_TRY(cudaMemcpyAsync(s->d_in, s->h_in, 4 * in_words, cudaMemcpyHostToDevice, s->stream));
    maz_search_call dc = *c;
    auto din = [&](size_t at) { return s->d_in + 4 * at; };
    dc.root_hidden = (const float *)din(o_hid);
    dc.rewards = (const float *)din(o_r);
    dc.values = (const float *)din(o_v);
    dc.logits = (const float *)din(o_log);
    dc.legal = c->legal ? (const float *)din(o_leg) : nullptr;
    dc.noise = (const float *)din(o_noi);
    dc.factor = c->factor ? (const int *)din(o_fac) : nullptr;
    size_t q = 0;
    auto take = [&](size_t words) { char *p = s->d_out + 4 * q; q += words; return p; };
    maz_search_readout &r = dc.out;
    r.values = (float *)take(n_b);
    r.marginal_visit_count = (int *)take(n_mv);
    r.marginal_priors = (float *)take(n_mv);
    r.num_children = (int *)take(n_b);
    r.actions = (int *)take(n_act);
    r.visit_count = (int *)take(n_k);
    float **f9[9] = {&r.pred_probs, &r.beta, &r.beta_hat, &r.priors, &r.imp_ratio, &r.pred_values, &r.mcts_values, &r.rewards, &r.qvalues};
    for (auto pf : f9) *pf = (float *)take(n_k);
    MAZ_TRY(maz_search_run_dev(s, &dc));
    CU_TRY(cudaMemcpyAsync(s->h_out, s->d_out, 4 * out_words, cudaMemcpyDeviceToHost, s->stream));
    MAZ_TRY(maz_search_check(s));
    const maz_search_readout &u = c->out;
    q = 0;
    auto give = [&](void *dst, size_t words) {
        if (dst) std::memcpy(dst, s->h_out + 4 * q, 4 * words);
        q += words;
    };
    give(u.values, n_b); give(u.marginal_visit_count, n_mv); give(u.marginal_priors, n_mv); give(u.num_children, n_b);
    give(u.actions, n_act); give(u.visit_count, n_k);
    float *uf[9] = {u.pred_probs, u.beta, u.beta_hat, u.priors, u.imp_ratio, u.pred_values, u.mcts_values, u.rewards, u.qvalues};
    for (float *p : uf) give(p, n_k);
    return MAZ_OK;
}
```

### mazero_b200/csrc/search_persist.cuh

```cuda
#pragma once
#include "infer_hmma.cuh"
#include "tree_step.cuh"

namespace maz {
namespace persist {

using namespace hmma;

struct SearchParams {
    Desc d;
    TreeLayout L;
    char *arena;
    const float *lam_pow, *logterm;
    const double *sqrtn;
    int table_len;
    float discount;
    int K, S;
    int *g_err;
    int *idx_y;
    int *greedy_w;
    float *rec_r, *rec_v, *rec_p, *rec_b;
    int *rec_ix, *rec_act;
    long long *tree_clock;
};

__device__ __forceinline__ unsigned long long globaltimer_ns()
{
    unsigned long long t;
    asm volatile("mov.u64 %0, %globaltimer;" : "=l"(t));
    return t;
}

constexpr uint32_t TREE_SCRATCH_OFF = OFF_PH;
constexpr uint32_t TREE_SCRATCH_BYTES = OFF_STAT - OFF_PH;

struct ExtraMap {
    uint32_t hot_stride;
    uint32_t o_qd, o_path, o_exp, o_dep;
    uint32_t o_xr, o_xv, o_xp, o_xb, o_xi, o_xa;
    uint32_t bytes;
};
__host__ __device__ inline uint32_t al16(uint32_t x) { return (x + 15u) & ~15u; }
__host__ __device__ inline ExtraMap extra_map(int rpt, int Nt, int A, int S)
{
    ExtraMap m;
    const uint32_t lv = (uint32_t)S + 2;
    m.o_qd = 64;
    m.o_path = m.o_qd + al16(4 * lv);
    m.o_exp = m.o_path + al16(2 * lv);
    m.o_dep = m.o_exp + al16(2 * lv);
    m.hot_stride = m.o_dep + al16(2 * lv);
    uint32_t o = m.hot_stride * (uint32_t)rpt;
    const uint32_t NA = (uint32_t)Nt * A;
    m.o_xr = o; o += al16(4 * rpt);
    m.o_xv = o; o += al16(4 * rpt);
    m.o_xp = o; o += al16(4 * rpt * NA);
    m.o_xb = o; o += al16(4 * rpt * NA);
    m.o_xi = o; o += al16(4 * rpt);
    m.o_xa = o; o += al16(4 * rpt * Nt);
    m.bytes = o;
    return m;
}
__host__ __device__ inline size_t persist_smem_bytes(int vec_floats, int rpt, int Nt, int A, int S)
{
    return ((smem_bytes(vec_floats) + 15) & ~(size_t)15) + extra_map(rpt, Nt, A, S).bytes;
}

__device__ __forceinline__ void gather_root(const Desc &d, int root, int rl, int ix, const int *tree_act, int lane)
{
    HSM_DECL;
    const int N = d.N;
#pragma unroll 1
    for (int j0 = 0; j0 < N; j0 += 4) {
        float4 v[4];
        int act[4];
#pragma unroll
        for (int u = 0; u < 4; ++u) {
            const int j = j0 + u;
            if (j < N) {
                v[u] = __ldcg(reinterpret_cast<const float4 *>(d.pool + ((size_t)ix * d.B + root) * (size_t)(N * H) + (size_t)j * H) + lane);
                if (d.greedy_pool == nullptr || d.cur < 0) act[u] = tree_act[j];
                else if (j == d.cur) act[u] = tree_act[0];
                else if (j < d.cur) act[u] = d.factor ? __ldcg(d.factor + (size_t)root * N + j) : 0;
                else act[u] = __ldcg(d.greedy_pool + ((size_t)ix * d.B + root) * N + j);
            }
        }
#pragma unroll
        for (int u = 0; u < 4; ++u) {
            const int j = j0 + u;
            if (j < N) {
                const int r = rl * N + j;
                *reinterpret_cast<uint2 *>(hsm + OFF_HH + (size_t)r * LDA + lane * 8) = make_uint2(pack2(v[u].x, v[u].y), pack2(v[u].z, v[u].w));
                if (2 * lane < d.KA)
                    *reinterpret_cast<uint32_t *>(hsm + OFF_ONE + (size_t)r * LDO + lane * 4) =
                        pack2((2 * lane == act[u]) ? 1.f : 0.f, (2 * lane + 1 == act[u]) ? 1.f : 0.f);
            }
        }
    }
}

constexpr int PERSIST_THREADS = NCONS + 128;
constexpr int REGS_COMPUTE = 232, REGS_PRODUCER = 40;

template <bool kProf>
__global__ void __launch_bounds__(PERSIST_THREADS, 1) k_search_persistent(const __grid_constant__ SearchParams P)
{
    HSM_DECL;
    __shared__ __align__(8) uint64_t bar_full[NSLOT], bar_empty[NSLOT], bar_vec;
    const Desc &d = P.d;
    const int tid = threadIdx.x, warp = tid >> 5, lane = tid & 31;

    if (tid == 0) {
        for (int i = 0; i < NSLOT; ++i) { mbar_init(&bar_full[i], 1); mbar_init(&bar_empty[i], NCONS / 32); }
        mbar_init(&bar_vec, 1);
        mbar_fence_init();
    }
    setup_rows(d);
    for (uint32_t o = tid * 16u; o < TM * (uint32_t)LDA + TM * (uint32_t)LDO; o += PERSIST_THREADS * 16u)
        *reinterpret_cast<uint4 *>(hsm + OFF_HH + o) = make_uint4(0u, 0u, 0u, 0u);
    __syncthreads();
    if (warp >= NCONS / 32) {
        asm volatile("setmaxnreg.dec.sync.aligned.u32 %0;" ::"n"(REGS_PRODUCER));
        if (warp == NCONS / 32 && lane == 0) produce_weights(d, bar_full, bar_empty, &bar_vec, P.S);
        return;
    }
    asm volatile("setmaxnreg.inc.sync.aligned.u32 %0;" ::"n"(REGS_COMPUTE));
    Ring ring{bar_full, bar_empty, 0};
    TreeLayout Lprof = P.L;
    if (kProf && P.tree_clock != nullptr)
        Lprof.dbg_clock = P.tree_clock + 2 * P.S + 4 * (long long)gridDim.x + 64 + 4 * (long long)P.d.B;
    const TreeLayout &L = kProf ? Lprof : P.L;
    const int rpt = tile_rpt(d);
    const int root0 = blockIdx.x * rpt;
    const int tree = root0 + warp;
    const bool has_tree = warp < rpt && tree < d.B;
    char *tb = P.arena + (size_t)(has_tree ? tree : 0) * L.slab_bytes;
    const size_t B = (size_t)d.B, NA = (size_t)L.N * L.A;
    const StepScratch scr = carve_step_scratch(reinterpret_cast<char *>(hsm) + TREE_SCRATCH_OFF + (size_t)warp * tree_scratch_bytes(L.N, L.A, L.K, L.S),
                                               L.N, L.A, L.K, L.S);
    const ExtraMap xm = extra_map(rpt, L.N, L.A, L.S);
    char *xbase = reinterpret_cast<char *>(hsm) + ((smem_bytes(d.vec_floats) + 15) & ~(size_t)15);
    char *hb = xbase + (size_t)(warp < rpt ? warp : 0) * xm.hot_stride;
    TreeHdr *hdr = reinterpret_cast<TreeHdr *>(hb);
    const TreeHot hot{reinterpret_cast<uint16_t *>(hb + xm.o_path), reinterpret_cast<float *>(hb + xm.o_qd),
                      reinterpret_cast<uint16_t *>(hb + xm.o_exp), reinterpret_cast<uint16_t *>(hb + xm.o_dep)};
    float *x_r = reinterpret_cast<float *>(xbase + xm.o_xr), *x_v = reinterpret_cast<float *>(xbase + xm.o_xv);
    float *x_p = reinterpret_cast<float *>(xbase + xm.o_xp), *x_b = reinterpret_cast<float *>(xbase + xm.o_xb);
    int *x_i = reinterpret_cast<int *>(xbase + xm.o_xi), *x_a = reinterpret_cast<int *>(xbase + xm.o_xa);
    if (has_tree) {
        const TreeHot g = hot_from_slab(L, tb);
        if (lane < 16) reinterpret_cast<int *>(hdr)[lane] = reinterpret_cast<const int *>(f_hdr(tb))[lane];
        for (int i = lane; i < L.S + 2; i += 32) {
            hot.path[i] = g.path[i]; hot.qd[i] = g.qd[i]; hot.expslot[i] = g.expslot[i]; hot.depth[i] = g.depth[i];
        }
    }
    __syncwarp();

    long long *clk = (kProf && P.tree_clock != nullptr && blockIdx.x == 0 && tid == 0) ? P.tree_clock : nullptr;
    long long *cta_clk = (kProf && P.tree_clock != nullptr && tid == 0) ? P.tree_clock + 2 * P.S + 4 * blockIdx.x : nullptr;
    const long long k0 = cta_clk ? clock64() : 0;
    const unsigned long long g0 = cta_clk ? globaltimer_ns() : 0;
    long long sum_inf = 0, sum_tree = 0;
    long long *tree_clk = (kProf && P.tree_clock != nullptr && has_tree && lane == 0)
                              ? P.tree_clock + 2 * P.S + 4 * (long long)gridDim.x + 64 + 4 * (long long)tree : nullptr;
    long long tc_eb = 0, tc_sel = 0, tc_len = 0, tc_max = 0;

    mbar_wait(&bar_vec, 0);
    setup_head_copies(d);
    cta_sync();

    SimIo io;
    io.idx_x = x_i; io.actions = x_a; io.reward = x_r; io.value = x_v; io.probs = x_p; io.beta = x_b; io.root0 = root0;
    io.logits_out = nullptr;

#pragma unroll 1
    for (int s = 0; s <= P.S; ++s) {
        const long long t1 = cta_clk ? clock64() : 0;
        if (has_tree) {
            const long long q0 = tree_clk ? clock64() : 0;
            if (s > 0) {
                if (P.rec_r != nullptr) {
                    const size_t o = (size_t)(s - 1) * B + tree;
                    if (lane == 0) { P.rec_r[o] = x_r[warp]; P.rec_v[o] = x_v[warp]; }
                    for (int t = lane; t < (int)NA; t += 32) {
                        P.rec_p[o * NA + t] = x_p[(size_t)warp * NA + t];
                        P.rec_b[o * NA + t] = x_b[(size_t)warp * NA + t];
                    }
                }
                expand_backup_device<false>(L, tb, hdr, hot, P.lam_pow, s, P.discount, P.K, x_r + warp, x_v + warp, x_p + (size_t)warp * NA,
                                            x_b + (size_t)warp * NA, scr, lane, P.g_err, kProf ? tree : -1);
            }
            __syncwarp();
            if (kProf && s > 0 && L.dbg_clock != nullptr && tree == 0 && lane == 0) {
                const int order[11] = {0, 1, 2, 11, 12, 13, 14, 15, 3, 4, 5};
                for (int i = 1; i < 11; ++i) L.dbg_clock[16 + i] += L.dbg_clock[order[i]] - L.dbg_clock[order[i - 1]];
            }
            const long long q1 = tree_clk ? clock64() : 0;
            if (s < P.S) {
                select_next_device(L, tb, hdr, hot, P.logterm, P.sqrtn, P.table_len, P.discount, warp, lane, &scr, x_i, nullptr, x_a,
                                   P.g_err);
                __syncwarp();
                const int ix = x_i[warp];
                if (P.rec_ix != nullptr) {
                    const size_t o = (size_t)s * B + tree;
                    if (lane == 0) P.rec_ix[o] = ix;
                    for (int j = lane; j < L.N; j += 32) P.rec_act[o * L.N + j] = x_a[warp * L.N + j];
                }
                gather_root(d, tree, warp, ix, x_a + warp * L.N, lane);
            }
            if (tree_clk) {
                const long long q2 = clock64();
                const int pl = hdr->path_len;
                tc_eb += q1 - q0; tc_sel += q2 - q1; tc_len += pl; tc_max = pl > tc_max ? pl : tc_max;
            }
        }
        cta_sync();
        const long long t2 = cta_clk ? clock64() : 0;
        if (cta_clk) {
            sum_tree += t2 - t1;
            if (clk && s > 0) clk[2 * (s - 1) + 1] = t2 - t1;
        }
        if (s == P.S) break;
        io.next_hidden = d.next_hidden + (size_t)s * B * (size_t)(d.N * H);
        io.greedy = P.greedy_w ? P.greedy_w + (size_t)(s + 1) * B * d.N : nullptr;
        long long *sclk = (clk && s == P.S / 2) ? P.tree_clock + 2 * P.S + 4 * (long long)gridDim.x : nullptr;
        if (sclk) { sclk[0] = t2; sclk[1] = t2; }
        infer_stages(d, io, ring, sclk);
        cta_sync();
        if (cta_clk) {
            const long long t3 = clock64();
            sum_inf += t3 - t2;
            if (clk) clk[2 * s] = t3 - t2;
        }
    }
    if (has_tree && lane < 16) reinterpret_cast<int *>(f_hdr(tb))[lane] = reinterpret_cast<const int *>(hdr)[lane];
    if (tree_clk) { tree_clk[0] = tc_eb; tree_clk[1] = tc_sel; tree_clk[2] = tc_len; tree_clk[3] = tc_max; }
    if (cta_clk) {
        cta_clk[0] = clock64() - k0;
        cta_clk[1] = (long long)(globaltimer_ns() - g0);
        cta_clk[2] = sum_inf;
        cta_clk[3] = sum_tree;
    }
}

}
}
```

### mazero_b200/fused.py

```python
import ctypes as C
import os

import torch

from ._lib import check, lib

NCHUNK = 32
SWIZZLE = False
H, GH, PH, SUP = 128, 64, 32, 11


class InferDesc(C.Structure):
    _fields_ = [
        ("B", C.c_int), ("N", C.c_int), ("A", C.c_int), ("KA", C.c_int), ("NAP", C.c_int), ("Nt", C.c_int), ("cur", C.c_int),
        ("inv_tau", C.c_float),
        ("pool", C.c_void_p), ("idx_x", C.c_void_p), ("actions", C.c_void_p), ("next_hidden", C.c_void_p),
        ("reward", C.c_void_p), ("value", C.c_void_p), ("probs", C.c_void_p), ("beta", C.c_void_p), ("greedy", C.c_void_p),
        ("logits_out", C.c_void_p), ("wpk", C.c_void_p), ("vec", C.c_void_p), ("vec_floats", C.c_int),
        ("chunk_off", C.c_uint * NCHUNK), ("chunk_bytes", C.c_uint * NCHUNK),
        ("o_bin", C.c_int), ("o_pos", C.c_int), ("o_layer", C.c_int), ("o_dyn", C.c_int), ("o_rg", C.c_int),
        ("o_vg", C.c_int), ("o_pol", C.c_int), ("dbg_clock", C.c_void_p), ("dbg_flags", C.c_int),
        ("roots_per_tile", C.c_int), ("factor", C.c_void_p), ("greedy_pool", C.c_void_p),
        ("tc_layout", C.c_int), ("o_oh_in", C.c_int), ("o_oh_dyn", C.c_int), ("o_oh_rg", C.c_int),
    ]


def _pad16(n):
    return (n + 15) // 16 * 16


def pack_operand(w):
    r, k = w.shape
    assert r % 8 == 0 and k % 16 == 0, (r, k)
    wb = w.to(torch.bfloat16)
    if SWIZZLE and k % 64 == 0:
        t = wb.view(r // 8, 8, k // 64, 8, 8).permute(2, 0, 1, 3, 4)
        ar = torch.arange(8, device=w.device)
        src_chunk = ar[None, :] ^ ar[:, None]
        return t[:, :, ar[:, None], src_chunk, :].contiguous().view(-1)
    return wb.view(r // 8, 8, k // 8, 8).permute(0, 2, 1, 3).contiguous().view(-1)


def pack_rowmajor(w):
    r, k = w.shape
    assert r % 16 == 0 and k % 16 == 0, (r, k)
    out = torch.zeros(r, k + 8, dtype=torch.bfloat16, device=w.device)
    out[:, :k] = w.to(torch.bfloat16)
    return out.view(-1)


def _interleave_gnn(stacked):
    nq = lib.maz_infer_small_nq()
    fw = GH // nq
    gc, nn = stacked[:GH], stacked[GH:]
    return torch.cat([torch.cat([gc[fw * q:fw * (q + 1)], nn[fw * q:fw * (q + 1)]]) for q in range(nq)])


def _padcols(w, k):
    out = torch.zeros(w.shape[0], k, dtype=w.dtype, device=w.device)
    out[:, : w.shape[1]] = w
    return out


def _padrows(w, r):
    out = torch.zeros(r, w.shape[1], dtype=w.dtype, device=w.device)
    out[: w.shape[0]] = w
    return out


def supported(sd, num_agents, action_space_size, hidden):
    d = "dynamics_network."
    try:
        return (hidden == H and num_agents <= 30 and action_space_size <= 48
                and f"{d}attention_stack.2.encoder.layers.2.linear1.weight" in sd
                and f"{d}attention_stack.2.encoder.layers.3.linear1.weight" not in sd
                and sd[f"{d}attention_stack.2.encoder.layers.0.linear1.weight"].shape == (H, H)
                and sd[f"{d}fc_dynamic.3.weight"].shape == (H, H) and f"{d}fc_dynamic.6.weight" in sd
                and f"{d}fc_dynamic.9.weight" not in sd
                and sd[f"{d}reward_predictor.gc1.lin_layer.weight"].shape[0] == GH
                and sd[f"{d}reward_predictor.V.weight"].shape[0] == SUP
                and sd["prediction_network.value_predictor.V.weight"].shape[0] == SUP
                and sd["prediction_network.fc_policy.0.weight"].shape[0] == PH
                and "prediction_network.fc_policy.3.weight" in sd and "prediction_network.fc_policy.6.weight" not in sd)
    except KeyError:
        return False


class FusedParams:

    def __init__(self, sd, num_agents, action_space_size, device):
        self.N, self.A = int(num_agents), int(action_space_size)
        self.KA = _pad16(self.A)
        self.device = torch.device(device)
        self.wpk = None
        self.vec = None
        self.repack(sd)

    def repack(self, sd):
        dev, N, A, KA = self.device, self.N, self.A, self.KA
        g = lambda k: sd[k].detach().to(device=dev, dtype=torch.float32)
        d, p = "dynamics_network.", "prediction_network."
        chunks = []
        w_in = g(d + "attention_stack.0.weight")
        chunks += [w_in[:, :H], _padcols(w_in[:, H:H + A], KA)]
        for l in range(3):
            e = f"{d}attention_stack.2.encoder.layers.{l}."
            qkv = g(e + "self_attn.in_proj_weight")
            chunks += [qkv[0:H], qkv[H:2 * H], qkv[2 * H:3 * H], g(e + "self_attn.out_proj.weight"),
                       g(e + "linear1.weight"), g(e + "linear2.weight")]
        wd1 = g(d + "fc_dynamic.0.weight")
        chunks += [wd1[:, :H], _padcols(wd1[:, H:H + A], KA), wd1[:, H + A:], g(d + "fc_dynamic.3.weight"),
                   g(d + "fc_dynamic.6.weight")]
        r = d + "reward_predictor."
        wr1 = torch.cat([g(r + "gc1.lin_layer.weight"), g(r + "nn_gc1.weight")], 0)
        chunks += [wr1[:, :H], _padcols(wr1[:, H:H + A], KA)]
        chunks.append(torch.cat([g(r + "gc2.lin_layer.weight"), g(r + "nn_gc2.weight")], 0))
        v = p + "value_predictor."
        chunks.append(torch.cat([g(v + "gc1.lin_layer.weight"), g(v + "nn_gc1.weight")], 0))
        chunks.append(torch.cat([g(v + "gc2.lin_layer.weight"), g(v + "nn_gc2.weight")], 0))
        chunks.append(g(p + "fc_policy.0.weight"))
        chunks.append(_padrows(g(p + "fc_policy.3.weight"), KA))
        assert len(chunks) == NCHUNK
        c = chunks
        hm = c[:25] + [_interleave_gnn(c[25]), _interleave_gnn(c[26]), _interleave_gnn(c[28]), c[30],
                       _interleave_gnn(c[27]), _interleave_gnn(c[29]), c[31]]
        hp = [pack_rowmajor(t.contiguous()) for t in hm]
        offs_h, o = [], 0
        for t in hp:
            offs_h.append(o)
            o += t.numel() * 2
        wpk_h = torch.cat(hp)
        self.chunk_off_h, self.chunk_bytes_h = offs_h, [t.numel() * 2 for t in hp]
        if getattr(self, "wpk_h", None) is None:
            self.wpk_h = wpk_h
        else:
            self.wpk_h.copy_(wpk_h)
        packed = [pack_operand(c.contiguous()) for c in chunks]
        offs, o = [], 0
        for t in packed:
            offs.append(o)
            o += t.numel() * 2
        wpk = torch.cat(packed)
        self.chunk_off = offs
        self.chunk_bytes = [t.numel() * 2 for t in packed]

        tw = [c[0]]
        for l in range(3):
            b = 2 + 6 * l
            wq, wk, wv = c[b], c[b + 1], c[b + 2]
            for h in (0, 1):
                tw += [torch.cat([wq[64 * h:64 * h + 64], wk[64 * h:64 * h + 64]], 0), wv[64 * h:64 * h + 64]]
            tw += [c[b + 3], c[b + 4], c[b + 5]]
        tw += [c[20], c[22], c[23], c[24], c[25], c[27], c[28], c[29], c[30], c[31]]
        assert len(tw) == NCHUNK
        tp = []
        for m in tw:
            m = m.contiguous()
            tp.append(torch.cat([pack_operand(m[:, k0:k0 + 64].contiguous()) for k0 in range(0, m.shape[1], 64)]))
        offs_t, o = [], 0
        for t in tp:
            offs_t.append(o)
            o += t.numel() * 2
        wpk_t = torch.cat(tp)
        self.chunk_off_t, self.chunk_bytes_t = offs_t, [t.numel() * 2 for t in tp]
        if getattr(self, "wpk_t", None) is None:
            self.wpk_t = wpk_t
        else:
            self.wpk_t.copy_(wpk_t)
        oh = [w[:, H:H + A].t().contiguous().to(torch.bfloat16).view(torch.float32) for w in (w_in, wd1, wr1)]

        vec, self.off = [], {}

        def put(name, *ts):
            self.off[name] = sum(t.numel() for t in vec)
            for t in ts:
                vec.append(t.reshape(-1))

        z16 = torch.zeros(16, device=dev)
        put("bin", g(d + "attention_stack.0.bias"))
        put("pos", g(d + "attention_stack.2.pos_embed.pos_table")[0, :N].contiguous())
        self.off["layer"] = sum(t.numel() for t in vec)
        for l in range(3):
            e = f"{d}attention_stack.2.encoder.layers.{l}."
            qb = g(e + "self_attn.in_proj_bias")
            vec += [qb, g(e + "self_attn.out_proj.bias"), g(e + "norm1.weight"), g(e + "norm1.bias"), g(e + "linear1.bias"),
                    g(e + "linear2.bias"), g(e + "norm2.weight"), g(e + "norm2.bias")]
        put("dyn", g(d + "fc_dynamic.0.bias"), g(d + "fc_dynamic.1.weight"), g(d + "fc_dynamic.1.bias"),
            g(d + "fc_dynamic.3.bias"), g(d + "fc_dynamic.4.weight"), g(d + "fc_dynamic.4.bias"), g(d + "fc_dynamic.6.bias"))
        for name, pre in (("rg", r), ("vg", v)):
            put(name, g(pre + "gc1.lin_layer.bias"), g(pre + "nn_gc1.bias"), g(pre + "gc2.lin_layer.bias"), g(pre + "nn_gc2.bias"),
                g(pre + "V.weight"), torch.cat([g(pre + "V.bias"), z16[: 16 - SUP]]))
        bp2 = torch.cat([g(p + "fc_policy.3.bias"), torch.zeros(KA - A, device=dev)])
        put("pol", g(p + "fc_policy.0.bias"), g(p + "fc_policy.1.weight"), g(p + "fc_policy.1.bias"), bp2)
        vecf = torch.cat(vec)
        if vecf.numel() % 8:
            vecf = torch.cat([vecf, torch.zeros(8 - vecf.numel() % 8, device=dev)])
        vecf = vecf.contiguous()
        assert all(o % 4 == 0 for o in self.off.values())
        self.off_oh = [vecf.numel() + i * A * (H // 2) for i in range(3)]
        vec_t = torch.cat([vecf] + [t.reshape(-1) for t in oh]).contiguous()
        if self.wpk is None:
            self.wpk, self.vec, self.vec_t = wpk, vecf, vec_t
        else:
            self.wpk.copy_(wpk)
            self.vec.copy_(vecf)
            self.vec_t.copy_(vec_t)

    def desc(self, B, pool, idx_x, actions, next_hidden, reward, value, probs, beta, greedy=None, logits_out=None,
             tree_agents=None, cur=-1, inv_tau=1.0, dbg_clock=None, small=False, factor=None, greedy_pool=None, roots_per_tile=0,
             twin=None):
        ptr = lambda t: (t.data_ptr() if t is not None else None)
        dsc = InferDesc()
        dsc.B, dsc.N, dsc.A, dsc.KA, dsc.NAP = int(B), self.N, self.A, self.KA, self.KA
        dsc.Nt = self.N if tree_agents is None else int(tree_agents)
        dsc.cur, dsc.inv_tau = int(cur), float(inv_tau)
        dsc.pool, dsc.idx_x, dsc.actions, dsc.next_hidden = ptr(pool), ptr(idx_x), ptr(actions), ptr(next_hidden)
        dsc.reward, dsc.value, dsc.probs, dsc.beta = ptr(reward), ptr(value), ptr(probs), ptr(beta)
        dsc.greedy, dsc.logits_out = ptr(greedy), ptr(logits_out)
        dsc.dbg_clock = ptr(dbg_clock)
        dsc.factor, dsc.greedy_pool, dsc.roots_per_tile = ptr(factor), ptr(greedy_pool), int(roots_per_tile)
        import os as _os
        dsc.dbg_flags = int(_os.environ.get('MAZ_DBG_FLAGS', '0'))
        twin = (not small) and (use_twin(B, self.N) if twin is None else bool(twin))
        dsc.wpk, dsc.vec, dsc.vec_floats = (self.wpk_h if small else self.wpk).data_ptr(), self.vec.data_ptr(), self.vec.numel()
        co, cb = (self.chunk_off_h, self.chunk_bytes_h) if small else (self.chunk_off, self.chunk_bytes)
        if twin:
            dsc.tc_layout = 1
            dsc.wpk, dsc.vec, dsc.vec_floats = self.wpk_t.data_ptr(), self.vec_t.data_ptr(), self.vec_t.numel()
            co, cb = self.chunk_off_t, self.chunk_bytes_t
            dsc.o_oh_in, dsc.o_oh_dyn, dsc.o_oh_rg = self.off_oh
        for i in range(NCHUNK):
            dsc.chunk_off[i], dsc.chunk_bytes[i] = co[i], cb[i]
        o = self.off
        dsc.o_bin, dsc.o_pos, dsc.o_layer, dsc.o_dyn = o["bin"], o["pos"], o["layer"], o["dyn"]
        dsc.o_rg, dsc.o_vg, dsc.o_pol = o["rg"], o["vg"], o["pol"]
        return dsc


def _weights_desc(self, B, small):
    return self.desc(B, None, None, None, None, None, None, None, None, small=small)


FusedParams.weights_desc = _weights_desc


SMALL_MAX_TILES = int(os.environ.get("MAZ_INFER_SMALL_MAX_TILES", "222"))


def use_twin(B=None, N=None):
    mode = os.environ.get("MAZ_INFER_TC", "auto")
    if mode in ("twin", "v1"):
        return mode == "twin"
    if B is None or N is None:
        return True
    sms = 148
    tiles = -(-int(B) // (4 * (32 // int(N))))
    pairs = (tiles + 1) // 2
    t_pairs = -(-pairs // sms) * (141.0 + 0.2 * int(N))
    t_tiles = -(-tiles // sms) * (80.0 + 3.2 * int(N))
    return t_pairs < t_tiles


def use_small(B, N):
    mode = os.environ.get("MAZ_INFER_KERNEL", "auto")
    if mode in ("small", "tcgen05"):
        return mode == "small"
    rpt = 32 // N
    return (B + rpt - 1) // rpt <= SMALL_MAX_TILES


def launch(dsc, stream_ptr, small=False):
    fn = lib.maz_infer_recurrent_small if small else lib.maz_infer_recurrent
    check(fn(C.byref(dsc), C.c_void_p(stream_ptr)))
```

Measured before the change: 18.14 million.

## Load MMA weight fragments directly from global/L1 instead of TMA smem ring

```diff
diff --git a/mazero_b200/csrc/infer_hmma.cuh b/mazero_b200/csrc/infer_hmma.cuh
--- a/mazero_b200/csrc/infer_hmma.cuh
+++ b/mazero_b200/csrc/infer_hmma.cuh
@@ -10,7 +10,7 @@
 using namespace umma;
 
 constexpr int H = 128, NHEAD = 8, HD = 16, GH = 64, PH = 32, SUP = 11, NLAYER = 3;
-constexpr int NCHUNK = MAZ_INFER_NCHUNK, NSLOT = 3;
+constexpr int NCHUNK = MAZ_INFER_NCHUNK;
 constexpr int TM = 32;
 #ifndef MAZ_HMMA_NQ
 #define MAZ_HMMA_NQ 4
@@ -20,7 +20,7 @@
 constexpr int GT = GH / NQ / 8;
 constexpr int CW = H / NQ, FW = GH / NQ;
 static_assert(NQ == 4 || NQ == 8, "NQ");
-constexpr int NCONS = 64 * NQ, NTHREADS = NCONS + 32;
+constexpr int NCONS = 64 * NQ, NTHREADS = NCONS;
 constexpr int PAD = 8;
 constexpr int LDA = (H + PAD) * 2;
 constexpr int LDQ = (3 * H + PAD) * 2;
@@ -28,15 +28,9 @@
 constexpr int LDO = (48 + PAD) * 2;
 constexpr int LDG = GH + 4;
 constexpr int LDV = GH + 4;
-constexpr uint32_t SLOT_BYTES = 128 * (H + PAD) * 2;
-#ifndef MAZ_HMMA_PIECE
-#define MAZ_HMMA_PIECE 4352
-#endif
-constexpr uint32_t PIECE = MAZ_HMMA_PIECE;
-#ifndef MAZ_GEMM_UNROLL
-#define MAZ_GEMM_UNROLL 2
-#endif
-constexpr int GEMM_UNROLL = MAZ_GEMM_UNROLL;
+constexpr uint32_t MAX_CHUNK_BYTES = H * H * 2;
+constexpr uint32_t WFRAG = 32 * 16;
+constexpr int PREFETCH_AHEAD = 3;
 
 constexpr uint32_t OFF_X = 0;
 constexpr uint32_t OFF_T = OFF_X + TM * LDA;
@@ -48,8 +42,7 @@
 constexpr uint32_t STAT_SET = TM * NQ * 8;
 constexpr uint32_t OFF_VP = OFF_STAT + 3 * TM * NQ * 8;
 constexpr uint32_t OFF_ROW = OFF_VP + 2 * SUP * LDV * 4;
-constexpr uint32_t OFF_W = ((OFF_ROW + TM * 16 + 127) / 128) * 128;
-constexpr uint32_t OFF_P = OFF_W + NSLOT * SLOT_BYTES;
+constexpr uint32_t OFF_P = ((OFF_ROW + TM * 16 + 127) / 128) * 128;
 constexpr int G_R = 0, G_V = TM * LDG;
 constexpr int Y_R = 0, Y_V = TM * GH;
 constexpr int PL0 = 2 * TM * LDG;
@@ -116,93 +109,78 @@
 
 struct Thr {
     int lane, warp, g, t, mt, nq, rA, rB;
-    uint32_t a_off, w_off;
+    uint32_t a_off;
     __device__ __forceinline__ Thr()
     {
         const int tid = threadIdx.x;
         lane = tid & 31; warp = tid >> 5; g = lane >> 2; t = lane & 3; mt = warp & 1; nq = warp >> 1;
         rA = 16 * mt + g; rB = rA + 8;
         a_off = (uint32_t)(16 * mt + (lane & 7) + ((lane >> 3) & 1) * 8);
-        w_off = (uint32_t)((lane & 7) + (lane >> 4) * 8);
     }
     __device__ __forceinline__ uint32_t a_addr(uint32_t tile, int lda) const { return tile + a_off * lda + (uint32_t)(lane >> 4) * 16u; }
-    __device__ __forceinline__ uint32_t w_addr(uint32_t slot, int ldw, int n0) const
-    {
-        return slot + (uint32_t)(n0 + w_off) * ldw + (uint32_t)((lane >> 3) & 1) * 16u;
-    }
 };
 
+__device__ __forceinline__ const uint8_t *chunk_ptr(const Desc &d, int k) { return reinterpret_cast<const uint8_t *>(d.wpk) + d.chunk_off[k]; }
+__device__ __forceinline__ uint4 ldw(const uint8_t *p) { return __ldg(reinterpret_cast<const uint4 *>(p)); }
+__device__ __forceinline__ void prefetch_chunk(const Desc &d, int k)
+{
+    k = k >= NCHUNK ? k - NCHUNK : k;
+    const uint32_t o = threadIdx.x * 128u;
+    if (o < d.chunk_bytes[k]) asm volatile("prefetch.global.L1 [%0];" ::"l"(chunk_ptr(d, k) + o));
+}
+__device__ __forceinline__ const uint8_t *take_chunk(const Desc &d, int k)
+{
+    prefetch_chunk(d, k + PREFETCH_AHEAD);
+    return chunk_ptr(d, k);
+}
+
+constexpr int BAHEAD = 4;
 template <int NT, int KS>
-__device__ __forceinline__ void gemm_fixed(float (&acc)[NT][4], const Thr &th, uint32_t a_tile, int lda, uint32_t w_slot, int ldw, int n0)
-{
-    const uint32_t aa = th.a_addr(a_tile, lda), wa = th.w_addr(w_slot, ldw, n0);
-    uint32_t a[2][4], b[2][NT / 2][4];
+__device__ __forceinline__ void gemm_fixed(float (&acc)[NT][4], const Thr &th, uint32_t a_tile, int lda, const uint8_t *w, int n0)
+{
+    const uint32_t aa = th.a_addr(a_tile, lda);
+    const uint8_t *wl = w + (size_t)(n0 / 16) * KS * WFRAG + th.lane * 16;
+    uint4 b[KS][NT / 2];
+#pragma unroll
+    for (int ks = 0; ks < KS && ks < BAHEAD; ++ks)
+#pragma unroll
+        for (int p = 0; p < NT / 2; ++p) b[ks][p] = ldw(wl + (p * KS + ks) * WFRAG);
+    uint32_t a[2][4];
     ldsm4(aa, a[0]);
 #pragma unroll
-    for (int p = 0; p < NT / 2; ++p) ldsm4(wa + (uint32_t)(16 * p) * ldw, b[0][p]);
-#pragma unroll GEMM_UNROLL
     for (int ks = 0; ks < KS; ++ks) {
-        const int cur = ks & 1, nxt = cur ^ 1;
-        if (ks + 1 < KS) {
-            ldsm4(aa + 32u * (ks + 1), a[nxt]);
-#pragma unroll
-            for (int p = 0; p < NT / 2; ++p) ldsm4(wa + (uint32_t)(16 * p) * ldw + 32u * (ks + 1), b[nxt][p]);
-        }
+        const int cur = ks & 1;
+        if (ks + BAHEAD < KS)
+#pragma unroll
+            for (int p = 0; p < NT / 2; ++p) b[ks + BAHEAD][p] = ldw(wl + (p * KS + ks + BAHEAD) * WFRAG);
+        if (ks + 1 < KS) ldsm4(aa + 32u * (ks + 1), a[cur ^ 1]);
 #pragma unroll
         for (int p = 0; p < NT / 2; ++p) {
-            mma16816(acc[2 * p], a[cur], b[cur][p][0], b[cur][p][1]);
-            mma16816(acc[2 * p + 1], a[cur], b[cur][p][2], b[cur][p][3]);
+            mma16816(acc[2 * p], a[cur], b[ks][p].x, b[ks][p].y);
+            mma16816(acc[2 * p + 1], a[cur], b[ks][p].z, b[ks][p].w);
         }
     }
 }
 template <int NT>
-__device__ __forceinline__ void gemm_rt(float (&acc)[NT][4], const Thr &th, uint32_t a_tile, int lda, uint32_t w_slot, int ldw, int n0, int K)
-{
-    const uint32_t aa = th.a_addr(a_tile, lda), wa = th.w_addr(w_slot, ldw, n0);
+__device__ __forceinline__ void gemm_rt(float (&acc)[NT][4], const Thr &th, uint32_t a_tile, int lda, const uint8_t *w, int n0, int K)
+{
+    const int KS = K / 16;
+    const uint32_t aa = th.a_addr(a_tile, lda);
+    const uint8_t *wl = w + (size_t)(n0 / 16) * KS * WFRAG + th.lane * 16;
 #pragma unroll 1
-    for (int k0 = 0; k0 < K; k0 += 16) {
-        uint32_t a[4], b[NT / 2][4];
-        ldsm4(aa + 2u * k0, a);
-#pragma unroll
-        for (int p = 0; p < NT / 2; ++p) ldsm4(wa + (uint32_t)(16 * p) * ldw + 2u * k0, b[p]);
+    for (int ks = 0; ks < KS; ++ks) {
+        uint4 b[NT / 2];
+#pragma unroll
+        for (int p = 0; p < NT / 2; ++p) b[p] = ldw(wl + (p * KS + ks) * WFRAG);
+        uint32_t a[4];
+        ldsm4(aa + 32u * ks, a);
 #pragma unroll
         for (int p = 0; p < NT / 2; ++p) {
-            mma16816(acc[2 * p], a, b[p][0], b[p][1]);
-            mma16816(acc[2 * p + 1], a, b[p][2], b[p][3]);
-        }
-    }
-}
-
-__device__ __forceinline__ void issue_chunk(const Desc &d, int k, int slot, uint64_t *bar_full)
-{
-    HSM_DECL;
-    const uint32_t nbytes = (d.dbg_flags & 4) ? 16u : d.chunk_bytes[k];
-    const uint8_t *src = reinterpret_cast<const uint8_t *>(d.wpk) + d.chunk_off[k];
-    uint8_t *dst = hsm + OFF_W + (size_t)slot * SLOT_BYTES;
-    mbar_expect_tx(&bar_full[slot], nbytes);
-    for (uint32_t o = 0; o < nbytes; o += PIECE) {
-        const uint32_t n = (nbytes - o < PIECE) ? (nbytes - o) : PIECE;
-        bulk_g2s(dst + o, src + o, n, &bar_full[slot]);
-    }
-}
-
-struct Ring {
-    uint64_t *full, *empty;
-    int c;
-    __device__ __forceinline__ uint32_t acquire(int ahead = 0)
-    {
-        const int cc = c + ahead, s = cc % NSLOT;
-        mbar_wait(&full[s], (cc / NSLOT) & 1);
-        return sbase() + OFF_W + (uint32_t)s * SLOT_BYTES;
-    }
-    __device__ __forceinline__ void release(int lane, int n = 1)
-    {
-        __syncwarp();
-        if (lane == 0)
-            for (int i = 0; i < n; ++i) mbar_arrive(&empty[(c + i) % NSLOT]);
-        c += n;
-    }
-};
+            mma16816(acc[2 * p], a, b[p].x, b[p].y);
+            mma16816(acc[2 * p + 1], a, b[p].z, b[p].w);
+        }
+    }
+}
 
 __device__ __forceinline__ void cta_sync() { named_bar_sync(1, NCONS); }
 
@@ -344,19 +322,15 @@
     }
 }
 
-static __device__ __noinline__ void stage_inproj(const Desc &d, Ring &ring, float (&xio)[NT][4])
+static __device__ __noinline__ void stage_inproj(const Desc &d, float (&xio)[NT][4])
 {
     const Thr th;
     const uint32_t sb = sbase();
-    const int n0 = CW * th.nq, ldo = (d.KA + PAD) * 2;
+    const int n0 = CW * th.nq;
     float x[NT][4];
     zero<NT>(x);
-    uint32_t w = ring.acquire();
-    gemm_fixed<NT, 8>(x, th, sb + OFF_HH, LDA, w, LDA, n0);
-    ring.release(th.lane);
-    w = ring.acquire();
-    gemm_rt<NT>(x, th, sb + OFF_ONE, LDO, w, ldo, n0, d.KA);
-    ring.release(th.lane);
+    gemm_fixed<NT, 8>(x, th, sb + OFF_HH, LDA, take_chunk(d, 0), n0);
+    gemm_rt<NT>(x, th, sb + OFF_ONE, LDO, take_chunk(d, 1), n0, d.KA);
     add_bias<NT>(x, th, sb + OFF_P + 4u * d.o_bin, n0);
     const uint32_t pA = sb + OFF_P + 4u * (d.o_pos + row_info(th.rA).agent * H), pB = sb + OFF_P + 4u * (d.o_pos + row_info(th.rB).agent * H);
 #pragma unroll
@@ -371,44 +345,21 @@
     cta_sync();
 }
 
-static __device__ __noinline__ void stage_qkv(Ring &ring, uint32_t lv)
+static __device__ __noinline__ void stage_qkv(const Desc &d, int k0, uint32_t lv)
 {
     const Thr th;
     const uint32_t sb = sbase();
     const int n0 = CW * th.nq;
-    float acc[3 * NT][4];
-    zero<3 * NT>(acc);
-    uint32_t wa[3];
-#pragma unroll
-    for (int i = 0; i < 3; ++i) wa[i] = th.w_addr(ring.acquire(i), LDA, n0);
-    const uint32_t aa = th.a_addr(sb + OFF_X, LDA);
-    constexpr int PW = NT / 2, NP = 3 * PW;
-    uint32_t a[2][4], b[2][NP][4];
-    ldsm4(aa, a[0]);
-#pragma unroll
-    for (int p = 0; p < NP; ++p) ldsm4(wa[p / PW] + (uint32_t)(16 * (p % PW)) * LDA, b[0][p]);
-#pragma unroll GEMM_UNROLL
-    for (int ks = 0; ks < 8; ++ks) {
-        const int cur = ks & 1, nxt = cur ^ 1;
-        if (ks + 1 < 8) {
-            ldsm4(aa + 32u * (ks + 1), a[nxt]);
-#pragma unroll
-            for (int p = 0; p < NP; ++p) ldsm4(wa[p / PW] + (uint32_t)(16 * (p % PW)) * LDA + 32u * (ks + 1), b[nxt][p]);
-        }
-#pragma unroll
-        for (int p = 0; p < NP; ++p) {
-            mma16816(acc[2 * p], a[cur], b[cur][p][0], b[cur][p][1]);
-            mma16816(acc[2 * p + 1], a[cur], b[cur][p][2], b[cur][p][3]);
-        }
-    }
-    ring.release(th.lane, 3);
-#pragma unroll
+#pragma unroll 1
     for (int which = 0; which < 3; ++which) {
+        float acc[NT][4];
+        zero<NT>(acc);
+        gemm_fixed<NT, 8>(acc, th, sb + OFF_X, LDA, take_chunk(d, k0 + which), n0);
 #pragma unroll
         for (int nt = 0; nt < NT; ++nt) {
             const int c = n0 + 8 * nt + 2 * th.t;
             const float2 bv = ldp2(lv + 4u * (which * H + c));
-            const float *v = acc[which * NT + nt];
+            const float *v = acc[nt];
             sts32(sb + OFF_Q + (uint32_t)th.rA * LDQ + 2u * (which * H + c), pack2(v[0] + bv.x, v[1] + bv.y));
             sts32(sb + OFF_Q + (uint32_t)th.rB * LDQ + 2u * (which * H + c), pack2(v[2] + bv.x, v[3] + bv.y));
         }
@@ -529,16 +480,14 @@
     cta_sync();
 }
 
-static __device__ __noinline__ void stage_residual_ln(Ring &ring, float (&xio)[NT][4], uint32_t bias, uint32_t gam, uint32_t bet)
+static __device__ __noinline__ void stage_residual_ln(const Desc &d, int k, float (&xio)[NT][4], uint32_t bias, uint32_t gam, uint32_t bet)
 {
     const Thr th;
     const uint32_t sb = sbase();
     const int n0 = CW * th.nq;
     float x[NT][4];
     copy<NT>(x, xio);
-    const uint32_t w = ring.acquire();
-    gemm_fixed<NT, 8>(x, th, sb + OFF_T, LDA, w, LDA, n0);
-    ring.release(th.lane);
+    gemm_fixed<NT, 8>(x, th, sb + OFF_T, LDA, take_chunk(d, k), n0);
     add_bias<NT>(x, th, bias, n0);
     layer_norm128(x, th, gam, bet, n0, false);
     store_tile<NT>(sb + OFF_X, LDA, th, n0, x);
@@ -546,47 +495,37 @@
     cta_sync();
 }
 
-static __device__ __noinline__ void stage_linear_relu(Ring &ring, uint32_t bias)
+static __device__ __noinline__ void stage_linear_relu(const Desc &d, int k, uint32_t bias)
 {
     const Thr th;
     const uint32_t sb = sbase();
     const int n0 = CW * th.nq;
     float acc[NT][4];
     zero<NT>(acc);
-    const uint32_t w = ring.acquire();
-    gemm_fixed<NT, 8>(acc, th, sb + OFF_X, LDA, w, LDA, n0);
-    ring.release(th.lane);
+    gemm_fixed<NT, 8>(acc, th, sb + OFF_X, LDA, take_chunk(d, k), n0);
     add_bias<NT>(acc, th, bias, n0);
     relu<NT>(acc);
     store_tile<NT>(sb + OFF_T, LDA, th, n0, acc);
     cta_sync();
 }
 
-static __device__ __noinline__ void stage_dynamics(const Desc &d, Ring &ring, const SimIo io)
+static __device__ __noinline__ void stage_dynamics(const Desc &d, const SimIo io)
 {
     const Thr th;
     const uint32_t sb = sbase();
-    const int n0 = CW * th.nq, ldo = (d.KA + PAD) * 2;
+    const int n0 = CW * th.nq;
     const uint32_t dv = sb + OFF_P + 4u * d.o_dyn;
     float acc[NT][4];
     zero<NT>(acc);
-    uint32_t w = ring.acquire();
-    gemm_fixed<NT, 8>(acc, th, sb + OFF_HH, LDA, w, LDA, n0);
-    ring.release(th.lane);
-    w = ring.acquire();
-    gemm_rt<NT>(acc, th, sb + OFF_ONE, LDO, w, ldo, n0, d.KA);
-    ring.release(th.lane);
-    w = ring.acquire();
-    gemm_fixed<NT, 8>(acc, th, sb + OFF_X, LDA, w, LDA, n0);
-    ring.release(th.lane);
+    gemm_fixed<NT, 8>(acc, th, sb + OFF_HH, LDA, take_chunk(d, 20), n0);
+    gemm_rt<NT>(acc, th, sb + OFF_ONE, LDO, take_chunk(d, 21), n0, d.KA);
+    gemm_fixed<NT, 8>(acc, th, sb + OFF_X, LDA, take_chunk(d, 22), n0);
     add_bias<NT>(acc, th, dv, n0);
     layer_norm128(acc, th, dv + 4u * 128, dv + 4u * 256, n0, true);
     store_tile<NT>(sb + OFF_T, LDA, th, n0, acc);
     cta_sync();
     zero<NT>(acc);
-    w = ring.acquire();
-    gemm_fixed<NT, 8>(acc, th, sb + OFF_T, LDA, w, LDA, n0);
-    ring.release(th.lane);
+    gemm_fixed<NT, 8>(acc, th, sb + OFF_T, LDA, take_chunk(d, 23), n0);
     add_bias<NT>(acc, th, dv + 4u * 384, n0);
     layer_norm128(acc, th, dv + 4u * 512, dv + 4u * 640, n0, true);
     store_tile<NT>(sb + OFF_X, LDA, th, n0, acc);
@@ -603,9 +542,7 @@
             hv[hf][nt] = ri.valid ? __ldcg(reinterpret_cast<const float2 *>(hp + n0 + 8 * nt + 2 * th.t)) : make_float2(0.f, 0.f);
     }
     zero<NT>(acc);
-    w = ring.acquire();
-    gemm_fixed<NT, 8>(acc, th, sb + OFF_X, LDA, w, LDA, n0);
-    ring.release(th.lane);
+    gemm_fixed<NT, 8>(acc, th, sb + OFF_X, LDA, take_chunk(d, 24), n0);
     add_bias<NT>(acc, th, dv + 4u * 768, n0);
 #pragma unroll
     for (int hf = 0; hf < 2; ++hf) {
@@ -684,25 +621,18 @@
     }
 }
 
-static __device__ __noinline__ void stage_heads1(const Desc &d, Ring &ring)
+static __device__ __noinline__ void stage_heads1(const Desc &d)
 {
     const Thr th;
     const uint32_t sb = sbase();
-    const int n0 = CW * th.nq, ldo = (d.KA + PAD) * 2;
+    const int n0 = CW * th.nq;
     float aR[NT][4], aV[NT][4], aP[2][4];
     zero<NT>(aR); zero<NT>(aV); zero<2>(aP);
-    uint32_t w = ring.acquire();
-    gemm_fixed<NT, 8>(aR, th, sb + OFF_T, LDA, w, LDA, n0);
-    ring.release(th.lane);
-    w = ring.acquire();
-    gemm_rt<NT>(aR, th, sb + OFF_ONE, LDO, w, ldo, n0, d.KA);
-    ring.release(th.lane);
-    w = ring.acquire();
-    gemm_fixed<NT, 8>(aV, th, sb + OFF_T, LDA, w, LDA, n0);
-    ring.release(th.lane);
-    w = ring.acquire();
-    if (th.nq < 2) gemm_fixed<2, 8>(aP, th, sb + OFF_T, LDA, w, LDA, 16 * th.nq);
-    ring.release(th.lane);
+    gemm_fixed<NT, 8>(aR, th, sb + OFF_T, LDA, take_chunk(d, 25), n0);
+    gemm_rt<NT>(aR, th, sb + OFF_ONE, LDO, take_chunk(d, 26), n0, d.KA);
+    gemm_fixed<NT, 8>(aV, th, sb + OFF_T, LDA, take_chunk(d, 27), n0);
+    const uint8_t *wp = take_chunk(d, 28);
+    if (th.nq < 2) gemm_fixed<2, 8>(aP, th, sb + OFF_T, LDA, wp, 16 * th.nq);
     const uint32_t G = sb + OFF_Q, stat = sb + OFF_STAT, pr = sb + OFF_P + 4u * d.o_rg, pvv = sb + OFF_P + 4u * d.o_vg;
     const uint32_t pp = sb + OFF_P + 4u * d.o_pol;
     gnn_phase_a(aR, th, G + 4u * G_R, pr);
@@ -758,11 +688,11 @@
     return out;
 }
 
-static __device__ __noinline__ void stage_heads2(const Desc &d, Ring &ring, const SimIo io, long long *hs_clk)
+static __device__ __noinline__ void stage_heads2(const Desc &d, const SimIo io, long long *hs_clk)
 {
     const Thr th;
     const uint32_t sb = sbase();
-    const int n0 = CW * th.nq, ldg = (GH + PAD) * 2;
+    const int n0 = CW * th.nq;
     const int N = d.N, A = d.A, tid = threadIdx.x;
     int hs_n = 40;
 #define HS() \
@@ -770,16 +700,11 @@
     HS();
     float aR[NT][4], aV[NT][4], aP[2][4];
     zero<NT>(aR); zero<NT>(aV); zero<2>(aP);
-    uint32_t w = ring.acquire();
-    gemm_fixed<NT, 4>(aR, th, sb + OFF_X, LDA, w, ldg, n0);
-    ring.release(th.lane);
-    w = ring.acquire();
-    gemm_fixed<NT, 4>(aV, th, sb + OFF_X + GH * 2, LDA, w, ldg, n0);
-    ring.release(th.lane);
-    w = ring.acquire();
+    gemm_fixed<NT, 4>(aR, th, sb + OFF_X, LDA, take_chunk(d, 29), n0);
+    gemm_fixed<NT, 4>(aV, th, sb + OFF_X + GH * 2, LDA, take_chunk(d, 30), n0);
+    const uint8_t *wp = take_chunk(d, 31);
     const int pc0 = 16 * th.nq;
-    if (pc0 < d.NAP) gemm_fixed<2, 2>(aP, th, sb + OFF_PH, LDP, w, LDP, pc0);
-    ring.release(th.lane);
+    if (pc0 < d.NAP) gemm_fixed<2, 2>(aP, th, sb + OFF_PH, LDP, wp, pc0);
     const uint32_t G = sb + OFF_Q, stat = sb + OFF_STAT, pr = sb + OFF_P + 4u * (d.o_rg + 128), pvv = sb + OFF_P + 4u * (d.o_vg + 128);
     const uint32_t PL = G + 4u * PL0;
     HS();
@@ -945,18 +870,14 @@
     }
 }
 
-__device__ __forceinline__ void produce_weights(const Desc &d, uint64_t *bar_full, uint64_t *bar_empty, uint64_t *bar_vec, int rounds)
+__device__ __forceinline__ void load_params(const Desc &d, uint64_t *bar_vec)
 {
     HSM_DECL;
-    mbar_expect_tx(bar_vec, (uint32_t)d.vec_floats * 4u);
-    bulk_g2s(hsm + OFF_P, d.vec, (uint32_t)d.vec_floats * 4u, bar_vec);
-    const int total = rounds * NCHUNK;
-#pragma unroll 1
-    for (int c = 0, k = 0; c < total; ++c, k = (k + 1 == NCHUNK) ? 0 : k + 1) {
-        const int s = c % NSLOT;
-        if (c >= NSLOT) mbar_wait_backoff(&bar_empty[s], ((c / NSLOT) - 1) & 1);
-        issue_chunk(d, k, s, bar_full);
-    }
+    if (threadIdx.x == 0) {
+        mbar_expect_tx(bar_vec, (uint32_t)d.vec_floats * 4u);
+        bulk_g2s(hsm + OFF_P, d.vec, (uint32_t)d.vec_floats * 4u, bar_vec);
+    }
+    for (int k = 0; k < PREFETCH_AHEAD; ++k) prefetch_chunk(d, k);
 }
 
 __device__ __forceinline__ void setup_head_copies(const Desc &d)
@@ -968,36 +889,37 @@
     }
 }
 
-__device__ __forceinline__ void infer_stages(const Desc &d, const SimIo io, Ring &ring, long long *clk)
+__device__ __forceinline__ void infer_stages(const Desc &d, const SimIo io, long long *clk)
 {
     int ts_n = 2;
 #define TS() \
     if (clk && ts_n < 64) clk[ts_n++] = clock64();
     TS();
     float x[NT][4];
-    stage_inproj(d, ring, x);
+    stage_inproj(d, x);
     TS();
     const uint32_t pbase = sbase() + OFF_P;
 #pragma unroll 1
     for (int l = 0; l < NLAYER; ++l) {
         const uint32_t lv = pbase + 4u * (d.o_layer + l * 1280);
-        stage_qkv(ring, lv);
+        const int k0 = 2 + 6 * l;
+        stage_qkv(d, k0, lv);
         TS();
         stage_attention(d);
         TS();
-        stage_residual_ln(ring, x, lv + 4u * 384, lv + 4u * 512, lv + 4u * 640);
+        stage_residual_ln(d, k0 + 3, x, lv + 4u * 384, lv + 4u * 512, lv + 4u * 640);
         TS();
-        stage_linear_relu(ring, lv + 4u * 768);
+        stage_linear_relu(d, k0 + 4, lv + 4u * 768);
         TS();
-        stage_residual_ln(ring, x, lv + 4u * 896, lv + 4u * 1024, lv + 4u * 1152);
+        stage_residual_ln(d, k0 + 5, x, lv + 4u * 896, lv + 4u * 1024, lv + 4u * 1152);
         TS();
     }
     TS();
-    stage_dynamics(d, ring, io);
+    stage_dynamics(d, io);
     TS();
-    stage_heads1(d, ring);
+    stage_heads1(d);
     TS();
-    stage_heads2(d, ring, io, clk);
+    stage_heads2(d, io, clk);
     TS();
 #undef TS
 }
@@ -1005,23 +927,16 @@
 #ifndef MAZ_HMMA_NO_KERNEL
 __global__ void __launch_bounds__(NTHREADS, 1) k_recurrent_inference_small(const __grid_constant__ Desc d)
 {
-    HSM_DECL;
-    __shared__ __align__(8) uint64_t bar_full[NSLOT], bar_empty[NSLOT], bar_vec;
-    const int tid = threadIdx.x, warp = tid >> 5;
+    __shared__ __align__(8) uint64_t bar_vec;
+    const int tid = threadIdx.x;
 
     if (tid == 0) {
-        for (int i = 0; i < NSLOT; ++i) { mbar_init(&bar_full[i], 1); mbar_init(&bar_empty[i], NCONS / 32); }
         mbar_init(&bar_vec, 1);
         mbar_fence_init();
     }
     setup_rows(d);
     __syncthreads();
-
-    if (warp == NCONS / 32) {
-        if ((tid & 31) == 0) produce_weights(d, bar_full, bar_empty, &bar_vec, 1);
-        return;
-    }
-    Ring ring{bar_full, bar_empty, 0};
+    load_params(d, &bar_vec);
     long long *clk = (d.dbg_clock != nullptr && blockIdx.x == 0 && tid == 0) ? d.dbg_clock : nullptr;
     if (clk) clk[0] = clock64();
     asm volatile("griddepcontrol.wait;" ::: "memory");
@@ -1032,7 +947,7 @@
     mbar_wait(&bar_vec, 0);
     setup_head_copies(d);
     cta_sync();
-    infer_stages(d, io, ring, clk);
+    infer_stages(d, io, clk);
 }
 #endif
 
diff --git a/mazero_b200/csrc/maz_infer.cu b/mazero_b200/csrc/maz_infer.cu
--- a/mazero_b200/csrc/maz_infer.cu
+++ b/mazero_b200/csrc/maz_infer.cu
@@ -137,6 +137,8 @@
     cudaError_t e = cudaFuncGetAttributes(&fa, hmma::k_recurrent_inference_small);
     if (e == cudaSuccess)
         e = cudaFuncSetAttribute(hmma::k_recurrent_inference_small, cudaFuncAttributeMaxDynamicSharedMemorySize, optin - (int)fa.sharedSizeBytes);
+    if (e == cudaSuccess)
+        e = cudaFuncSetAttribute(hmma::k_recurrent_inference_small, cudaFuncAttributePreferredSharedMemoryCarveout, cudaSharedmemCarveoutMaxL1);
     if (e == cudaSuccess) e = cudaFuncGetAttributes(&fa, fused::k_recurrent_inference);
     if (e == cudaSuccess)
         e = cudaFuncSetAttribute(fused::k_recurrent_inference, cudaFuncAttributeMaxDynamicSharedMemorySize, optin - (int)fa.sharedSizeBytes);
@@ -157,7 +159,7 @@
         return set_last_error(1, "maz_infer_recurrent_small: NULL tensor");
     if (d->vec_floats <= 0 || d->vec_floats % 4) return set_last_error(1, "maz_infer_recurrent_small: vec_floats must be a positive multiple of 4");
     for (int c = 0; c < MAZ_INFER_NCHUNK; ++c)
-        if (d->chunk_bytes[c] == 0 || d->chunk_bytes[c] > hmma::SLOT_BYTES || d->chunk_bytes[c] % 16 || d->chunk_off[c] % 16)
+        if (d->chunk_bytes[c] == 0 || d->chunk_bytes[c] > hmma::MAX_CHUNK_BYTES || d->chunk_bytes[c] % hmma::WFRAG || d->chunk_off[c] % 16)
             return set_last_error(1, "maz_infer_recurrent_small: bad weight chunk table");
     const size_t dyn = hmma::smem_bytes(d->vec_floats);
     if (dyn > 227 * 1024) return set_last_error(3, "maz_infer_recurrent_small: parameters do not fit in shared memory");
diff --git a/mazero_b200/csrc/maz_search.cu b/mazero_b200/csrc/maz_search.cu
--- a/mazero_b200/csrc/maz_search.cu
+++ b/mazero_b200/csrc/maz_search.cu
@@ -192,6 +192,8 @@
             e = cudaFuncSetAttribute(persist::k_search_persistent<false>, cudaFuncAttributeMaxDynamicSharedMemorySize, optin - (int)fa.sharedSizeBytes);
         if (e == cudaSuccess)
             e = cudaFuncSetAttribute(persist::k_search_persistent<true>, cudaFuncAttributeMaxDynamicSharedMemorySize, optin - (int)fa.sharedSizeBytes);
+        for (auto k : {persist::k_search_persistent<false>, persist::k_search_persistent<true>})
+            if (e == cudaSuccess) e = cudaFuncSetAttribute(k, cudaFuncAttributePreferredSharedMemoryCarveout, cudaSharedmemCarveoutMaxL1);
         if (e != cudaSuccess) {
             set_last_error(MAZ_ERR_CUDA, std::string("cudaFuncSetAttribute(k_search_persistent): ") + cudaGetErrorString(e));
             return fail(MAZ_ERR_CUDA);
diff --git a/mazero_b200/csrc/search_persist.cuh b/mazero_b200/csrc/search_persist.cuh
--- a/mazero_b200/csrc/search_persist.cuh
+++ b/mazero_b200/csrc/search_persist.cuh
@@ -99,19 +99,17 @@
     }
 }
 
-constexpr int PERSIST_THREADS = NCONS + 128;
-constexpr int REGS_COMPUTE = 232, REGS_PRODUCER = 40;
+constexpr int PERSIST_THREADS = NCONS;
 
 template <bool kProf>
 __global__ void __launch_bounds__(PERSIST_THREADS, 1) k_search_persistent(const __grid_constant__ SearchParams P)
 {
     HSM_DECL;
-    __shared__ __align__(8) uint64_t bar_full[NSLOT], bar_empty[NSLOT], bar_vec;
+    __shared__ __align__(8) uint64_t bar_vec;
     const Desc &d = P.d;
     const int tid = threadIdx.x, warp = tid >> 5, lane = tid & 31;
 
     if (tid == 0) {
-        for (int i = 0; i < NSLOT; ++i) { mbar_init(&bar_full[i], 1); mbar_init(&bar_empty[i], NCONS / 32); }
         mbar_init(&bar_vec, 1);
         mbar_fence_init();
     }
@@ -119,13 +117,7 @@
     for (uint32_t o = tid * 16u; o < TM * (uint32_t)LDA + TM * (uint32_t)LDO; o += PERSIST_THREADS * 16u)
         *reinterpret_cast<uint4 *>(hsm + OFF_HH + o) = make_uint4(0u, 0u, 0u, 0u);
     __syncthreads();
-    if (warp >= NCONS / 32) {
-        asm volatile("setmaxnreg.dec.sync.aligned.u32 %0;" ::"n"(REGS_PRODUCER));
-        if (warp == NCONS / 32 && lane == 0) produce_weights(d, bar_full, bar_empty, &bar_vec, P.S);
-        return;
-    }
-    asm volatile("setmaxnreg.inc.sync.aligned.u32 %0;" ::"n"(REGS_COMPUTE));
-    Ring ring{bar_full, bar_empty, 0};
+    load_params(d, &bar_vec);
     TreeLayout Lprof = P.L;
     if (kProf && P.tree_clock != nullptr)
         Lprof.dbg_clock = P.tree_clock + 2 * P.S + 4 * (long long)gridDim.x + 64 + 4 * (long long)P.d.B;
@@ -225,7 +217,7 @@
         io.greedy = P.greedy_w ? P.greedy_w + (size_t)(s + 1) * B * d.N : nullptr;
         long long *sclk = (clk && s == P.S / 2) ? P.tree_clock + 2 * P.S + 4 * (long long)gridDim.x : nullptr;
         if (sclk) { sclk[0] = t2; sclk[1] = t2; }
-        infer_stages(d, io, ring, sclk);
+        infer_stages(d, io, sclk);
         cta_sync();
         if (cta_clk) {
             const long long t3 = clock64();
diff --git a/mazero_b200/fused.py b/mazero_b200/fused.py
--- a/mazero_b200/fused.py
+++ b/mazero_b200/fused.py
@@ -41,12 +41,11 @@
     return wb.view(r // 8, 8, k // 8, 8).permute(0, 2, 1, 3).contiguous().view(-1)
 
 
-def pack_rowmajor(w):
+def pack_fragments(w):
     r, k = w.shape
     assert r % 16 == 0 and k % 16 == 0, (r, k)
-    out = torch.zeros(r, k + 8, dtype=torch.bfloat16, device=w.device)
-    out[:, :k] = w.to(torch.bfloat16)
-    return out.view(-1)
+    t = w.to(torch.bfloat16).view(r // 16, 2, 8, k // 16, 2, 4, 2)
+    return t.permute(0, 3, 2, 5, 1, 4, 6).contiguous().view(-1)
 
 
 def _interleave_gnn(stacked):
@@ -54,6 +53,37 @@
     fw = GH // nq
     gc, nn = stacked[:GH], stacked[GH:]
     return torch.cat([torch.cat([gc[fw * q:fw * (q + 1)], nn[fw * q:fw * (q + 1)]]) for q in range(nq)])
+
+
+def weight_chunks(g, A, KA):
+    d, p = "dynamics_network.", "prediction_network."
+    chunks = []
+    w_in = g(d + "attention_stack.0.weight")
+    chunks += [w_in[:, :H], _padcols(w_in[:, H:H + A], KA)]
+    for l in range(3):
+        e = f"{d}attention_stack.2.encoder.layers.{l}."
+        qkv = g(e + "self_attn.in_proj_weight")
+        chunks += [qkv[0:H], qkv[H:2 * H], qkv[2 * H:3 * H], g(e + "self_attn.out_proj.weight"),
+                   g(e + "linear1.weight"), g(e + "linear2.weight")]
+    wd1 = g(d + "fc_dynamic.0.weight")
+    chunks += [wd1[:, :H], _padcols(wd1[:, H:H + A], KA), wd1[:, H + A:], g(d + "fc_dynamic.3.weight"),
+               g(d + "fc_dynamic.6.weight")]
+    r = d + "reward_predictor."
+    wr1 = torch.cat([g(r + "gc1.lin_layer.weight"), g(r + "nn_gc1.weight")], 0)
+    chunks += [wr1[:, :H], _padcols(wr1[:, H:H + A], KA)]
+    chunks.append(torch.cat([g(r + "gc2.lin_layer.weight"), g(r + "nn_gc2.weight")], 0))
+    v = p + "value_predictor."
+    chunks.append(torch.cat([g(v + "gc1.lin_layer.weight"), g(v + "nn_gc1.weight")], 0))
+    chunks.append(torch.cat([g(v + "gc2.lin_layer.weight"), g(v + "nn_gc2.weight")], 0))
+    chunks.append(g(p + "fc_policy.0.weight"))
+    chunks.append(_padrows(g(p + "fc_policy.3.weight"), KA))
+    assert len(chunks) == NCHUNK
+    return chunks, (w_in, wd1, wr1)
+
+
+def small_chunks(c):
+    return c[:25] + [_interleave_gnn(c[25]), _interleave_gnn(c[26]), _interleave_gnn(c[28]), c[30],
+                     _interleave_gnn(c[27]), _interleave_gnn(c[29]), c[31]]
 
 
 def _padcols(w, k):
@@ -100,31 +130,10 @@
         dev, N, A, KA = self.device, self.N, self.A, self.KA
         g = lambda k: sd[k].detach().to(device=dev, dtype=torch.float32)
         d, p = "dynamics_network.", "prediction_network."
-        chunks = []
-        w_in = g(d + "attention_stack.0.weight")
-        chunks += [w_in[:, :H], _padcols(w_in[:, H:H + A], KA)]
-        for l in range(3):
-            e = f"{d}attention_stack.2.encoder.layers.{l}."
-            qkv = g(e + "self_attn.in_proj_weight")
-            chunks += [qkv[0:H], qkv[H:2 * H], qkv[2 * H:3 * H], g(e + "self_attn.out_proj.weight"),
-                       g(e + "linear1.weight"), g(e + "linear2.weight")]
-        wd1 = g(d + "fc_dynamic.0.weight")
-        chunks += [wd1[:, :H], _padcols(wd1[:, H:H + A], KA), wd1[:, H + A:], g(d + "fc_dynamic.3.weight"),
-                   g(d + "fc_dynamic.6.weight")]
-        r = d + "reward_predictor."
-        wr1 = torch.cat([g(r + "gc1.lin_layer.weight"), g(r + "nn_gc1.weight")], 0)
-        chunks += [wr1[:, :H], _padcols(wr1[:, H:H + A], KA)]
-        chunks.append(torch.cat([g(r + "gc2.lin_layer.weight"), g(r + "nn_gc2.weight")], 0))
-        v = p + "value_predictor."
-        chunks.append(torch.cat([g(v + "gc1.lin_layer.weight"), g(v + "nn_gc1.weight")], 0))
-        chunks.append(torch.cat([g(v + "gc2.lin_layer.weight"), g(v + "nn_gc2.weight")], 0))
-        chunks.append(g(p + "fc_policy.0.weight"))
-        chunks.append(_padrows(g(p + "fc_policy.3.weight"), KA))
-        assert len(chunks) == NCHUNK
+        r, v = d + "reward_predictor.", p + "value_predictor."
+        chunks, (w_in, wd1, wr1) = weight_chunks(g, A, KA)
         c = chunks
-        hm = c[:25] + [_interleave_gnn(c[25]), _interleave_gnn(c[26]), _interleave_gnn(c[28]), c[30],
-                       _interleave_gnn(c[27]), _interleave_gnn(c[29]), c[31]]
-        hp = [pack_rowmajor(t.contiguous()) for t in hm]
+        hp = [pack_fragments(t.contiguous()) for t in small_chunks(c)]
         offs_h, o = [], 0
         for t in hp:
             offs_h.append(o)
```

After: 17.73 million, median of 6. 0.978x the previous value.
